# edouardoyallon/acco

Hardware: NVIDIA H100
Metric: tokens/sec (device-timed, max over ranks) Llama ACCO bf16 sharded-Adam, 8x1024 tokens per GPU per micro-batch (higher is better)
Workload: dtype bf16

## Files before the change

### acco_b200/csrc/bindings.cpp

```cpp
#include <torch/extension.h>
#include <ATen/cuda/CUDAContext.h>
#include <c10/cuda/CUDAGuard.h>
#include <cuda_runtime.h>

#include <cmath>
#include <cstdlib>
#include <vector>

extern "C" {
int acco_norm_grid(int T, int H, int sms, int backward);
int acco_rmsnorm_fwd(const void* a, const void* r, const void* w, void* y, void* h, float* rstd, int T, int H, float eps,
                     int grid, cudaStream_t st);
int acco_rmsnorm_bwd(const void* dy, const void* dh_extra, const void* h, const void* w, const float* rstd, void* dh,
                     float* dw_partial, float* dw_out, void* dw_accum_bf16, int T, int H, int grid, cudaStream_t st);
int acco_rope_pack_bwd(const void* dq, const void* dk, const void* dv, const long long* strides, void* dqkv, const float* cos_t,
                       const float* sin_t, int B, int S, int Hq, int Hk, int D, int sms, cudaStream_t st);
int acco_rope_qkv(void* qkv, const float* cos_t, const float* sin_t, int T, int S, int n_rot, int n_total, int D, int inverse,
                  int sms, cudaStream_t st);
int acco_swiglu_fwd(const void* gu, void* out, long long T, int I, int sms, cudaStream_t st);
int acco_swiglu_bwd(const void* dout, const void* gu, void* dgu, long long T, int I, int sms, cudaStream_t st);
int acco_ce_fwd(const void* logits, const long long* labels, float* lse, float* row_loss, float* loss, float* inv_n, long long T,
                int V, int Vp, long long ignore_index, cudaStream_t st);
int acco_ce_bwd(void* logits, const long long* labels, const float* lse, const float* scale, long long T, int V, int Vp,
                long long ignore_index, cudaStream_t st);
int acco_layernorm_grid(int T, int H, int sms, int backward);
int acco_layernorm_fwd(const void* a, const void* r, const void* w, const void* b, void* y, void* h, float* mean, float* rstd, int T, int H,
                       float eps, int grid, cudaStream_t st);
int acco_layernorm_bwd(const void* dy, const void* dh_extra, const void* h, const void* w, const float* mean, const float* rstd, void* dh,
                       float* partial, float* dwdb_out, void* dw_accum_bf16, void* db_accum_bf16, int T, int H, int grid, cudaStream_t st);
int acco_gelu_fwd(const void* x, void* y, long long n, int sms, cudaStream_t st);
int acco_gelu_bwd(const void* dy, const void* x, void* dx, long long n, int sms, cudaStream_t st);
int acco_debug_occupy(unsigned long long ns, int ctas, float* sink, cudaStream_t st);
int acco_round_params_size();
int acco_gemm_run(const void* a, long long lda, int a_mn, const void* b, long long ldb, int b_mn, void* d, long long ldd, const void* bias,
                  int M, int N, int K, int accumulate, int bn_req, int splits_req, int pm_req, int pn_req, int msub_req, int sms, cudaStream_t st);
int acco_gemm_tn_gather(const void* x, const void* w_local, void* y, int M, int N, int K, const void* const* peers, int n_peers,
                        const int* tile_owner, uint32_t* flags, uint32_t* epoch, uint32_t* done, int sms, cudaStream_t st);
long long acco_gemm_map_encodes();
int acco_gemm_max_clusters(int cl, int sms);
void acco_gemm_set_debug(unsigned long long* buf);
void acco_gemm_choose(int M, int N, int K, int a_mn, int b_mn, int accumulate, int sms, int* out5);
int acco_gemm_tile_n();
int acco_gemm_tile_k();
int acco_attn_supported(int B, int S, int Hq, int Hk, int D, float scale);
int acco_attn_fwd(const void* q, const void* k, const void* v, long long ld, void* o, long long ld_o, float* lse, int B, int S, int Hq, int Hk,
                  int D, float scale, int window, const int* seg, cudaStream_t st);
int acco_attn_bwd(const void* q, const void* k, const void* v, long long ld, const void* o, long long ld_o, const void* d_o, long long ld_do,
                  const float* lse, float* delta, float* dq_acc, void* dk, void* dv, int B, int S, int Hq, int Hk, int D, float scale, int window,
                  const int* seg, cudaStream_t st);
}

namespace {

constexpr int kMaxWorld = 16;
struct RoundParams {
    const void* acc_peer[kMaxWorld];
    void* theta_peer[kMaxWorld];
    uint32_t* pad_peer[kMaxWorld];
    const void* acc_mc;
    void* theta_mc;
    float* master;
    float* exp_avg;
    float* exp_avg_sq;
    float* stash;
    int* stash_count;
    int* total_out;
    uint32_t* epoch;
    uint32_t* done_ctas;
    const float* inv_count_in;
    const long long* skip;
    int n_skip;
    int watchdog_s;
    int gated;
    long long slice;
    int rank, world, local_count;
    float lr, beta1, beta2, eps, weight_decay, bc1, bc2_rsqrt;
    int commit, add_stash, write_stash;
};
extern "C" int acco_rs_adam_ag(const RoundParams* P, int grad_bf16, int out_bf16, int mode, int grid, cudaStream_t st);
extern "C" int acco_round_norm(const RoundParams* P, int grad_bf16, int mode, int grid, float max_norm, float* out, cudaStream_t st);

int sm_count() {
    static int n = 0;
    if (!n) n = at::cuda::getCurrentDeviceProperties()->multiProcessorCount;
    return n;
}
cudaStream_t stream() { return at::cuda::getCurrentCUDAStream().stream(); }

void check_bf16(const torch::Tensor& t, const char* name) {
    TORCH_CHECK(t.is_cuda() && t.scalar_type() == torch::kBFloat16 && t.is_contiguous(), name, " must be a contiguous CUDA bf16 tensor");
}
void check_f32(const torch::Tensor& t, const char* name) {
    TORCH_CHECK(t.is_cuda() && t.scalar_type() == torch::kFloat32 && t.is_contiguous(), name, " must be a contiguous CUDA fp32 tensor");
}

std::vector<torch::Tensor> rmsnorm_fwd(torch::Tensor x, torch::Tensor w, double eps) {
    check_bf16(x, "x"); check_bf16(w, "weight");
    const c10::cuda::CUDAGuard guard(x.device());
    const int T = x.size(0), H = x.size(1);
    auto y = torch::empty_like(x);
    auto rstd = torch::empty({T}, x.options().dtype(torch::kFloat32));
    const int grid = acco_norm_grid(T, H, sm_count(), 0);
    TORCH_CHECK(acco_rmsnorm_fwd(x.data_ptr(), nullptr, w.data_ptr(), y.data_ptr(), nullptr, rstd.data_ptr<float>(), T, H, (float)eps, grid, stream()) == 0,
                "rmsnorm_fwd: unsupported hidden size ", H);
    return {y, rstd};
}

std::vector<torch::Tensor> add_rmsnorm_fwd(torch::Tensor a, torch::Tensor r, torch::Tensor w, double eps) {
    check_bf16(a, "a"); check_bf16(r, "r"); check_bf16(w, "weight");
    const c10::cuda::CUDAGuard guard(a.device());
    const int T = a.size(0), H = a.size(1);
    auto y = torch::empty_like(a);
    auto h = torch::empty_like(a);
    auto rstd = torch::empty({T}, a.options().dtype(torch::kFloat32));
    const int grid = acco_norm_grid(T, H, sm_count(), 0);
    TORCH_CHECK(acco_rmsnorm_fwd(a.data_ptr(), r.data_ptr(), w.data_ptr(), y.data_ptr(), h.data_ptr(), rstd.data_ptr<float>(), T, H, (float)eps, grid, stream()) == 0,
                "add_rmsnorm_fwd: unsupported hidden size ", H);
    return {y, h, rstd};
}

std::vector<torch::Tensor> norm_bwd_impl(torch::Tensor dy, const torch::Tensor* de, torch::Tensor h, torch::Tensor w, torch::Tensor rstd,
                                         c10::optional<torch::Tensor> wgrad) {
    check_bf16(dy, "dy"); check_bf16(h, "h"); check_bf16(w, "weight"); check_f32(rstd, "rstd");
    const c10::cuda::CUDAGuard guard(dy.device());
    const int T = dy.size(0), H = dy.size(1);
    auto dh = torch::empty_like(dy);
    const int grid = acco_norm_grid(T, H, sm_count(), 1);
    auto partial = torch::empty({grid, H}, dy.options().dtype(torch::kFloat32));
    torch::Tensor dw;
    void* accum = nullptr;
    if (wgrad.has_value() && wgrad->defined()) {
        check_bf16(*wgrad, "weight.grad");
        TORCH_CHECK(wgrad->numel() == H, "weight.grad has the wrong size");
        accum = wgrad->data_ptr();
        dw = torch::empty({0}, dy.options().dtype(torch::kFloat32));
    } else {
        dw = torch::empty({H}, dy.options().dtype(torch::kFloat32));
    }
    TORCH_CHECK(acco_rmsnorm_bwd(dy.data_ptr(), de ? de->data_ptr() : nullptr, h.data_ptr(), w.data_ptr(), rstd.data_ptr<float>(), dh.data_ptr(),
                                 partial.data_ptr<float>(), accum ? nullptr : dw.data_ptr<float>(), accum, T, H, grid, stream()) == 0,
                "rmsnorm_bwd: unsupported hidden size ", H);
    return {dh, dw};
}
std::vector<torch::Tensor> rmsnorm_bwd(torch::Tensor dy, torch::Tensor x, torch::Tensor w, torch::Tensor rstd, c10::optional<torch::Tensor> wgrad) {
    return norm_bwd_impl(dy, nullptr, x, w, rstd, wgrad);
}
std::vector<torch::Tensor> add_rmsnorm_bwd(torch::Tensor dy, torch::Tensor dh_extra, torch::Tensor h, torch::Tensor w, torch::Tensor rstd,
                                           c10::optional<torch::Tensor> wgrad) {
    check_bf16(dh_extra, "dh_extra");
    return norm_bwd_impl(dy, &dh_extra, h, w, rstd, wgrad);
}

std::vector<torch::Tensor> layernorm_fwd(torch::Tensor a, c10::optional<torch::Tensor> r, torch::Tensor w, torch::Tensor b, double eps) {
    check_bf16(a, "a"); check_bf16(w, "weight"); check_bf16(b, "bias");
    const bool has_r = r.has_value() && r->defined();
    if (has_r) check_bf16(*r, "r");
    const c10::cuda::CUDAGuard guard(a.device());
    const int T = a.size(0), H = a.size(1);
    TORCH_CHECK(w.numel() == H && b.numel() == H, "layernorm: weight/bias size");
    auto y = torch::empty_like(a);
    auto f32 = a.options().dtype(torch::kFloat32);
    auto mean = torch::empty({T}, f32), rstd = torch::empty({T}, f32);
    torch::Tensor h = has_r ? torch::empty_like(a) : torch::Tensor();
    const int grid = acco_layernorm_grid(T, H, sm_count(), 0);
    TORCH_CHECK(acco_layernorm_fwd(a.data_ptr(), has_r ? r->data_ptr() : nullptr, w.data_ptr(), b.data_ptr(), y.data_ptr(), has_r ? h.data_ptr() : nullptr,
                                   mean.data_ptr<float>(), rstd.data_ptr<float>(), T, H, (float)eps, grid, stream()) == 0,
                "layernorm_fwd: unsupported hidden size ", H);
    if (has_r) return {y, h, mean, rstd};
    return {y, mean, rstd};
}

std::vector<torch::Tensor> layernorm_bwd(torch::Tensor dy, c10::optional<torch::Tensor> dh_extra, torch::Tensor h, torch::Tensor w, torch::Tensor mean,
                                         torch::Tensor rstd, c10::optional<torch::Tensor> wgrad, c10::optional<torch::Tensor> bgrad) {
    check_bf16(dy, "dy"); check_bf16(h, "h"); check_bf16(w, "weight"); check_f32(mean, "mean"); check_f32(rstd, "rstd");
    const bool has_e = dh_extra.has_value() && dh_extra->defined();
    if (has_e) check_bf16(*dh_extra, "dh_extra");
    const c10::cuda::CUDAGuard guard(dy.device());
    const int T = dy.size(0), H = dy.size(1);
    auto dh = torch::empty_like(dy);
    const int grid = acco_layernorm_grid(T, H, sm_count(), 1);
    auto f32 = dy.options().dtype(torch::kFloat32);
    auto partial = torch::empty({grid, 2 * H}, f32);
    const bool accum = wgrad.has_value() && wgrad->defined() && bgrad.has_value() && bgrad->defined();
    torch::Tensor dwdb;
    if (accum) {
        check_bf16(*wgrad, "weight.grad"); check_bf16(*bgrad, "bias.grad");
        TORCH_CHECK(wgrad->numel() == H && bgrad->numel() == H, "grad sizes");
        dwdb = torch::empty({0}, f32);
    } else {
        dwdb = torch::empty({2 * H}, f32);
    }
    TORCH_CHECK(acco_layernorm_bwd(dy.data_ptr(), has_e ? dh_extra->data_ptr() : nullptr, h.data_ptr(), w.data_ptr(), mean.data_ptr<float>(),
                                   rstd.data_ptr<float>(), dh.data_ptr(), partial.data_ptr<float>(), accum ? nullptr : dwdb.data_ptr<float>(),
                                   accum ? wgrad->data_ptr() : nullptr, accum ? bgrad->data_ptr() : nullptr, T, H, grid, stream()) == 0,
                "layernorm_bwd: unsupported hidden size ", H);
    return {dh, dwdb};
}

torch::Tensor gelu_fwd(torch::Tensor x) {
    check_bf16(x, "x");
    const c10::cuda::CUDAGuard guard(x.device());
    auto y = torch::empty_like(x);
    TORCH_CHECK(acco_gelu_fwd(x.data_ptr(), y.data_ptr(), x.numel(), sm_count(), stream()) == 0, "gelu: numel must be a multiple of 8");
    return y;
}
torch::Tensor gelu_bwd(torch::Tensor dy, torch::Tensor x) {
    check_bf16(x, "x"); check_bf16(dy, "dy");
    const c10::cuda::CUDAGuard guard(x.device());
    auto dx = torch::empty_like(x);
    TORCH_CHECK(acco_gelu_bwd(dy.data_ptr(), x.data_ptr(), dx.data_ptr(), x.numel(), sm_count(), stream()) == 0, "gelu: numel must be a multiple of 8");
    return dx;
}

void rope_qkv_inplace(torch::Tensor qkv, torch::Tensor cos_t, torch::Tensor sin_t, int64_t B, int64_t S, int64_t n_rot,
                      int64_t n_total, int64_t D, bool inverse) {
    check_bf16(qkv, "qkv"); check_f32(cos_t, "cos"); check_f32(sin_t, "sin");
    const c10::cuda::CUDAGuard guard(qkv.device());
    TORCH_CHECK(qkv.numel() == B * S * n_total * D, "qkv has the wrong number of elements");
    TORCH_CHECK(cos_t.size(0) >= S && cos_t.size(1) == D / 2, "cos/sin tables must be [>=S, D/2]");
    TORCH_CHECK(acco_rope_qkv(qkv.data_ptr(), cos_t.data_ptr<float>(), sin_t.data_ptr<float>(), (int)(B * S), (int)S, (int)n_rot,
                              (int)n_total, (int)D, inverse ? 1 : 0, sm_count(), stream()) == 0,
                "rope: head_dim must be a multiple of 16");
}

torch::Tensor rope_pack_bwd(torch::Tensor dq, torch::Tensor dk, torch::Tensor dv, torch::Tensor cos_t, torch::Tensor sin_t) {
    TORCH_CHECK(dq.is_cuda() && dq.scalar_type() == torch::kBFloat16 && dk.scalar_type() == torch::kBFloat16 && dv.scalar_type() == torch::kBFloat16, "bf16 CUDA grads expected");
    TORCH_CHECK(dq.stride(3) == 1 && dk.stride(3) == 1 && dv.stride(3) == 1, "head dim must be contiguous");
    check_f32(cos_t, "cos"); check_f32(sin_t, "sin");
    const c10::cuda::CUDAGuard guard(dq.device());
    const int64_t B = dq.size(0), S = dq.size(1), Hq = dq.size(2), D = dq.size(3), Hk = dk.size(2);
    for (auto* t : {&dq, &dk, &dv}) TORCH_CHECK((t->stride(0) % 8 == 0) && (t->stride(1) % 8 == 0) && (t->stride(2) % 8 == 0) && ((uintptr_t)t->data_ptr() % 16 == 0), "16-byte aligned strides required");
    auto out = torch::empty({B * S, (Hq + 2 * Hk) * D}, dq.options());
    long long st[9] = {dq.stride(0), dq.stride(1), dq.stride(2), dk.stride(0), dk.stride(1), dk.stride(2), dv.stride(0), dv.stride(1), dv.stride(2)};
    TORCH_CHECK(acco_rope_pack_bwd(dq.data_ptr(), dk.data_ptr(), dv.data_ptr(), st, out.data_ptr(), cos_t.data_ptr<float>(), sin_t.data_ptr<float>(),
                                   (int)B, (int)S, (int)Hq, (int)Hk, (int)D, sm_count(), stream()) == 0, "rope_pack_bwd: head_dim must be a multiple of 16");
    return out;
}

torch::Tensor swiglu_fwd(torch::Tensor gu) {
    check_bf16(gu, "gate_up");
    const c10::cuda::CUDAGuard guard(gu.device());
    const int64_t T = gu.size(0), I = gu.size(1) / 2;
    auto out = torch::empty({T, I}, gu.options());
    TORCH_CHECK(acco_swiglu_fwd(gu.data_ptr(), out.data_ptr(), T, (int)I, sm_count(), stream()) == 0, "swiglu: I must be a multiple of 8");
    return out;
}

torch::Tensor swiglu_bwd(torch::Tensor dout, torch::Tensor gu) {
    check_bf16(dout, "dout"); check_bf16(gu, "gate_up");
    const c10::cuda::CUDAGuard guard(gu.device());
    const int64_t T = gu.size(0), I = gu.size(1) / 2;
    auto dgu = torch::empty_like(gu);
    TORCH_CHECK(acco_swiglu_bwd(dout.data_ptr(), gu.data_ptr(), dgu.data_ptr(), T, (int)I, sm_count(), stream()) == 0, "swiglu: I must be a multiple of 8");
    return dgu;
}

std::vector<torch::Tensor> ce_fwd(torch::Tensor logits, torch::Tensor labels, int64_t V, int64_t ignore_index) {
    check_bf16(logits, "logits");
    TORCH_CHECK(labels.is_cuda() && labels.scalar_type() == torch::kInt64 && labels.is_contiguous(), "labels must be contiguous CUDA int64");
    const c10::cuda::CUDAGuard guard(logits.device());
    const int64_t T = logits.size(0), Vp = logits.size(1);
    TORCH_CHECK(labels.numel() == T, "labels/logits row mismatch");
    auto f32 = logits.options().dtype(torch::kFloat32);
    auto lse = torch::empty({T}, f32);
    auto row_loss = torch::empty({T}, f32);
    auto loss = torch::empty({}, f32);
    auto inv_n = torch::empty({1}, f32);
    TORCH_CHECK(acco_ce_fwd(logits.data_ptr(), (const long long*)labels.data_ptr<int64_t>(), lse.data_ptr<float>(), row_loss.data_ptr<float>(),
                            loss.data_ptr<float>(), inv_n.data_ptr<float>(), T, (int)V, (int)Vp, ignore_index, stream()) == 0,
                "ce_fwd: padded vocab must be a multiple of 8 and >= V");
    return {loss, inv_n, lse};
}

void ce_bwd_inplace(torch::Tensor logits, torch::Tensor labels, torch::Tensor lse, torch::Tensor scale, int64_t V, int64_t ignore_index) {
    check_bf16(logits, "logits"); check_f32(lse, "lse"); check_f32(scale, "scale");
    const c10::cuda::CUDAGuard guard(logits.device());
    const int64_t T = logits.size(0), Vp = logits.size(1);
    TORCH_CHECK(acco_ce_bwd(logits.data_ptr(), (const long long*)labels.data_ptr<int64_t>(), lse.data_ptr<float>(), scale.data_ptr<float>(), T,
                            (int)V, (int)Vp, ignore_index, stream()) == 0, "ce_bwd: bad shapes");
}

int default_grid(int mode, long long slice) {
    const long long vec = slice / 8;
    long long want = (vec + 255) / 256;
    long long cap = mode == 0 ? (long long)sm_count() * 4 : (long long)sm_count();
    if (want < 1) want = 1;
    return (int)std::min(want, cap);
}

void fill_hyper(RoundParams& P, double lr, double b1, double b2, double eps, double wd, int64_t step, int64_t commit, bool add_stash, bool write_stash) {
    P.lr = (float)lr; P.beta1 = (float)b1; P.beta2 = (float)b2; P.eps = (float)eps; P.weight_decay = (float)wd;
    P.bc1 = (float)(1.0 - std::pow(b1, (double)step));
    P.bc2_rsqrt = (float)(1.0 / std::sqrt(1.0 - std::pow(b2, (double)step)));
    P.commit = (int)commit; P.add_stash = add_stash ? 1 : 0; P.write_stash = write_stash ? 1 : 0;
}

void adamw_shard(torch::Tensor grad_sum, torch::Tensor master, torch::Tensor exp_avg, torch::Tensor exp_avg_sq, torch::Tensor stash,
                 torch::Tensor out, torch::Tensor inv_count, torch::Tensor scratch ,
                 double lr, double b1, double b2, double eps, double wd, int64_t step, int64_t commit, bool add_stash, bool write_stash) {
    check_f32(master, "master"); check_f32(exp_avg, "exp_avg"); check_f32(exp_avg_sq, "exp_avg_sq"); check_f32(stash, "stash"); check_f32(inv_count, "inv_count");
    const c10::cuda::CUDAGuard guard(master.device());
    const int64_t S = master.numel();
    TORCH_CHECK(S % 8 == 0, "shard size must be a multiple of 8 (use slice alignment >= 8)");
    TORCH_CHECK(grad_sum.numel() >= S && out.numel() >= S && grad_sum.is_contiguous() && out.is_contiguous(), "bad grad/out");
    TORCH_CHECK(scratch.scalar_type() == torch::kInt32 && scratch.numel() >= 4, "scratch must be int32[4]");
    const bool gb = grad_sum.scalar_type() == torch::kBFloat16, ob = out.scalar_type() == torch::kBFloat16;
    TORCH_CHECK(gb || grad_sum.scalar_type() == torch::kFloat32, "grad dtype");
    TORCH_CHECK(ob || out.scalar_type() == torch::kFloat32, "out dtype");
    RoundParams P{};
    P.acc_peer[0] = grad_sum.data_ptr();
    P.theta_peer[0] = out.data_ptr();
    P.master = master.data_ptr<float>(); P.exp_avg = exp_avg.data_ptr<float>(); P.exp_avg_sq = exp_avg_sq.data_ptr<float>(); P.stash = stash.data_ptr<float>();
    int* sc = scratch.data_ptr<int>();
    P.stash_count = sc; P.total_out = sc + 1; P.epoch = (uint32_t*)(sc + 2); P.done_ctas = (uint32_t*)(sc + 3);
    P.inv_count_in = inv_count.data_ptr<float>();
    P.slice = S; P.rank = 0; P.world = 1; P.local_count = 0;
    fill_hyper(P, lr, b1, b2, eps, wd, step, commit, add_stash, write_stash);
    TORCH_CHECK(acco_rs_adam_ag(&P, gb, ob, 0, default_grid(0, S), stream()) == 0, "adamw_shard launch failed");
}

RoundParams round_params(const std::vector<int64_t>& acc_ptrs, const std::vector<int64_t>& theta_ptrs, const std::vector<int64_t>& pad_ptrs,
                         int64_t acc_mc, int64_t theta_mc, const torch::Tensor& stash, const torch::Tensor& scratch, int64_t slice, int64_t rank,
                         int64_t world, int64_t local_count, int64_t mode) {
    check_f32(stash, "stash");
    TORCH_CHECK(world >= 1 && world <= kMaxWorld, "world size out of range");
    TORCH_CHECK(mode >= 0 && mode <= 2, "mode must be 0 (local), 1 (p2p) or 2 (multimem)");
    TORCH_CHECK((int64_t)acc_ptrs.size() >= (mode == 0 ? 1 : world), "peer pointer table too short");
    TORCH_CHECK(mode == 0 || (int64_t)pad_ptrs.size() >= world, "signal pad table too short");
    TORCH_CHECK(slice % 8 == 0 && stash.numel() == slice, "slice must be a multiple of 8 and match the shard state");
    TORCH_CHECK(mode != 2 || acc_mc != 0, "multicast mode needs multicast pointers");
    TORCH_CHECK(scratch.scalar_type() == torch::kInt32 && scratch.numel() >= 4, "scratch must be int32[4]");
    RoundParams P{};
    for (size_t i = 0; i < acc_ptrs.size() && i < (size_t)kMaxWorld; ++i) P.acc_peer[i] = (const void*)acc_ptrs[i];
    for (size_t i = 0; i < theta_ptrs.size() && i < (size_t)kMaxWorld; ++i) P.theta_peer[i] = (void*)theta_ptrs[i];
    for (size_t i = 0; i < pad_ptrs.size() && i < (size_t)kMaxWorld; ++i) P.pad_peer[i] = (uint32_t*)pad_ptrs[i];
    P.acc_mc = (const void*)acc_mc; P.theta_mc = (void*)theta_mc;
    P.stash = stash.data_ptr<float>();
    int* sc = scratch.data_ptr<int>();
    P.stash_count = sc; P.total_out = sc + 1; P.epoch = (uint32_t*)(sc + 2); P.done_ctas = (uint32_t*)(sc + 3);
    P.inv_count_in = nullptr;
    P.slice = slice; P.rank = (int)rank; P.world = (int)world; P.local_count = (int)local_count;
    static int watchdog = -1;
    if (watchdog < 0) { const char* e = std::getenv("ACCO_ROUND_WATCHDOG_S"); watchdog = e ? std::atoi(e) : 1800; }
    P.watchdog_s = watchdog;
    static int gated = -1;
    if (gated < 0) { const char* e = std::getenv("ACCO_ROUND_GATE"); gated = (e && e[0] == '0') ? 0 : 1; }
    P.gated = mode != 0 ? gated : 0;
    return P;
}

void rs_adam_ag(std::vector<int64_t> acc_ptrs, std::vector<int64_t> theta_ptrs, std::vector<int64_t> pad_ptrs, int64_t acc_mc, int64_t theta_mc,
                torch::Tensor master, torch::Tensor exp_avg, torch::Tensor exp_avg_sq, torch::Tensor stash,
                torch::Tensor scratch , int64_t slice, int64_t rank, int64_t world, int64_t local_count,
                double lr, double b1, double b2, double eps, double wd, int64_t step, int64_t commit, bool add_stash, bool write_stash,
                bool grad_bf16, bool out_bf16, int64_t mode, int64_t grid, c10::optional<torch::Tensor> skip_ranges,
                c10::optional<torch::Tensor> inv_count) {
    check_f32(master, "master"); check_f32(exp_avg, "exp_avg"); check_f32(exp_avg_sq, "exp_avg_sq");
    const c10::cuda::CUDAGuard guard(master.device());
    TORCH_CHECK(master.numel() == slice, "slice must match the shard state");
    TORCH_CHECK((int64_t)theta_ptrs.size() >= (mode == 0 ? 1 : world), "peer pointer tables too short");
    TORCH_CHECK(mode != 2 || theta_mc != 0, "multicast mode needs multicast pointers");
    RoundParams P = round_params(acc_ptrs, theta_ptrs, pad_ptrs, acc_mc, theta_mc, stash, scratch, slice, rank, world, local_count, mode);
    P.master = master.data_ptr<float>(); P.exp_avg = exp_avg.data_ptr<float>(); P.exp_avg_sq = exp_avg_sq.data_ptr<float>();
    if (skip_ranges.has_value() && skip_ranges->defined() && skip_ranges->numel() > 0) {
        TORCH_CHECK(skip_ranges->is_cuda() && skip_ranges->scalar_type() == torch::kInt64 && skip_ranges->is_contiguous() && skip_ranges->numel() % 2 == 0,
                    "skip_ranges must be a contiguous CUDA int64 [n, 2] tensor");
        P.skip = (const long long*)skip_ranges->data_ptr<int64_t>();
        P.n_skip = (int)(skip_ranges->numel() / 2);
    }
    if (inv_count.has_value() && inv_count->defined()) {
        check_f32(*inv_count, "inv_count");
        TORCH_CHECK(inv_count->numel() >= 2, "inv_count must be the scratch of round_norm (inv_eff at index 1)");
        P.inv_count_in = inv_count->data_ptr<float>() + 1;
        if (mode != 0) P.gated = 2;
    }
    fill_hyper(P, lr, b1, b2, eps, wd, step, commit, add_stash, write_stash);
    const int g = grid > 0 ? (int)grid : default_grid((int)mode, slice);
    TORCH_CHECK(acco_rs_adam_ag(&P, grad_bf16, out_bf16, (int)mode, g, stream()) == 0, "rs_adam_ag launch failed");
}

void round_norm(std::vector<int64_t> acc_ptrs, std::vector<int64_t> pad_ptrs, int64_t acc_mc, torch::Tensor stash, torch::Tensor scratch,
                torch::Tensor out, int64_t slice, int64_t rank, int64_t world, int64_t local_count, bool add_stash, bool grad_bf16, int64_t mode,
                int64_t grid, double max_norm) {
    check_f32(out, "out");
    const c10::cuda::CUDAGuard guard(stash.device());
    TORCH_CHECK(max_norm > 0, "max_norm must be positive");
    RoundParams P = round_params(acc_ptrs, std::vector<int64_t>(), pad_ptrs, acc_mc, 0, stash, scratch, slice, rank, world, local_count, mode);
    P.add_stash = add_stash ? 1 : 0;
    const int g = grid > 0 ? (int)grid : default_grid((int)mode, slice);
    TORCH_CHECK(out.numel() >= 3 + g, "out must hold 3 + grid floats (", 3 + g, ")");
    TORCH_CHECK(acco_round_norm(&P, grad_bf16, (int)mode, g, (float)max_norm, out.data_ptr<float>(), stream()) == 0, "round_norm launch failed");
}

torch::Tensor gemm_tn(torch::Tensor x, torch::Tensor w, std::vector<int64_t> peer_ptrs, c10::optional<torch::Tensor> tile_owner,
                      c10::optional<torch::Tensor> flags, c10::optional<torch::Tensor> state, int64_t max_ctas) {
    check_bf16(x, "x"); check_bf16(w, "w");
    TORCH_CHECK(x.dim() == 2 && w.dim() == 2 && x.size(1) == w.size(1), "gemm_tn: x [M,K], w [N,K]");
    const c10::cuda::CUDAGuard guard(x.device());
    const int64_t M = x.size(0), K = x.size(1), N = w.size(0);
    TORCH_CHECK(K % 8 == 0 && N % 8 == 0, "gemm_tn: K and N must be multiples of 8");
    TORCH_CHECK((uintptr_t)x.data_ptr() % 16 == 0 && (uintptr_t)w.data_ptr() % 16 == 0, "gemm_tn: 16-byte aligned operands required");
    auto y = torch::empty({M, N}, x.options());
    const void* peers[8] = {nullptr};
    const int n_peers = (int)peer_ptrs.size();
    TORCH_CHECK(n_peers <= 8, "gemm_tn: at most 8 peers");
    const int* owner = nullptr; uint32_t* fl = nullptr; uint32_t* ep = nullptr; uint32_t* dn = nullptr;
    if (n_peers > 0) {
        TORCH_CHECK(tile_owner.has_value() && flags.has_value() && state.has_value(), "gather mode needs tile_owner, flags and state");
        const int64_t num_n = (N + acco_gemm_tile_n() - 1) / acco_gemm_tile_n(), num_k = (K + acco_gemm_tile_k() - 1) / acco_gemm_tile_k();
        TORCH_CHECK(tile_owner->scalar_type() == torch::kInt32 && tile_owner->numel() >= num_n && tile_owner->is_cuda(), "tile_owner: int32 CUDA [num_n]");
        TORCH_CHECK(flags->scalar_type() == torch::kInt32 && flags->numel() >= num_n * num_k * 2 && flags->is_cuda(), "flags: int32 CUDA [num_n*num_k*2]");
        TORCH_CHECK(state->scalar_type() == torch::kInt32 && state->numel() >= 2 && state->is_cuda(), "state: int32 CUDA [2]");
        for (int i = 0; i < n_peers; ++i) peers[i] = (const void*)peer_ptrs[i];
        owner = tile_owner->data_ptr<int>();
        fl = (uint32_t*)flags->data_ptr<int>();
        ep = (uint32_t*)state->data_ptr<int>();
        dn = ep + 1;
    }
    int sms = sm_count();
    if (max_ctas > 0 && max_ctas < sms) sms = (int)max_ctas;
    int rc;
    if (n_peers > 0)
        rc = acco_gemm_tn_gather(x.data_ptr(), w.data_ptr(), y.data_ptr(), (int)M, (int)N, (int)K, peers, n_peers, owner, fl, ep, dn, sms, stream());
    else
        rc = acco_gemm_run(x.data_ptr(), K, 0, w.data_ptr(), K, 0, y.data_ptr(), N, nullptr, (int)M, (int)N, (int)K, 0, 0, 0, 0, 0, 0, sms, stream());
    TORCH_CHECK(rc == 0, "gemm_tn launch failed, code ", rc);
    return y;
}

torch::Tensor gemm(torch::Tensor a, torch::Tensor b, c10::optional<torch::Tensor> out, c10::optional<torch::Tensor> bias, bool a_mn, bool b_mn,
                   bool accumulate, int64_t bn, int64_t splits, int64_t pm, int64_t pn, int64_t msub, int64_t max_ctas) {
    auto ok2d = [](const torch::Tensor& t) {
        return t.is_cuda() && t.scalar_type() == torch::kBFloat16 && t.dim() == 2 && t.stride(1) == 1 && t.stride(0) % 8 == 0 && t.stride(0) >= t.size(1) &&
               (uintptr_t)t.data_ptr() % 16 == 0;
    };
    TORCH_CHECK(ok2d(a) && ok2d(b), "gemm: operands must be 2-D CUDA bf16, unit inner stride, 16-byte aligned rows");
    const c10::cuda::CUDAGuard guard(a.device());
    const int64_t M = a_mn ? a.size(1) : a.size(0), K = a_mn ? a.size(0) : a.size(1);
    const int64_t N = b_mn ? b.size(1) : b.size(0), Kb = b_mn ? b.size(0) : b.size(1);
    TORCH_CHECK(K == Kb, "gemm: contraction sizes differ (", K, " vs ", Kb, ")");
    TORCH_CHECK(N % 8 == 0, "gemm: N must be a multiple of 8");
    torch::Tensor y;
    if (out.has_value() && out->defined()) {
        y = *out;
        TORCH_CHECK(ok2d(y) && y.size(0) == M && y.size(1) == N, "gemm: out must be a [M,N] CUDA bf16 matrix");
    } else {
        TORCH_CHECK(!accumulate, "gemm: accumulate needs `out`");
        y = torch::empty({M, N}, a.options());
    }
    const void* bias_p = nullptr;
    if (bias.has_value() && bias->defined()) {
        TORCH_CHECK(bias->is_cuda() && bias->scalar_type() == torch::kBFloat16 && bias->is_contiguous() && bias->numel() == N &&
                    (uintptr_t)bias->data_ptr() % 16 == 0, "gemm: bias must be a contiguous, 16-byte aligned CUDA bf16 [N] vector");
        bias_p = bias->data_ptr();
    }
    int sms = sm_count();
    if (max_ctas > 0 && max_ctas < sms) sms = (int)max_ctas;
    const int rc = acco_gemm_run(a.data_ptr(), a.stride(0), a_mn ? 1 : 0, b.data_ptr(), b.stride(0), b_mn ? 1 : 0, y.data_ptr(), y.stride(0), bias_p,
                             (int)M, (int)N, (int)K, accumulate ? 1 : 0, (int)bn, (int)splits, (int)pm, (int)pn, (int)msub, sms, stream());
    TORCH_CHECK(rc == 0, "gemm launch failed, code ", rc, " (M=", M, " N=", N, " K=", K, ")");
    return y;
}

std::vector<int64_t> gemm_choose(int64_t M, int64_t N, int64_t K, bool a_mn, bool b_mn, bool accumulate) {
    int o[5] = {0, 0, 0, 0, 0};
    acco_gemm_choose((int)M, (int)N, (int)K, a_mn ? 1 : 0, b_mn ? 1 : 0, accumulate ? 1 : 0, sm_count(), o);
    return {o[0], o[1], o[2], o[3], o[4]};
}
int64_t gemm_map_encodes() { return acco_gemm_map_encodes(); }
void gemm_set_debug(c10::optional<torch::Tensor> buf) {
    if (buf.has_value() && buf->defined()) {
        TORCH_CHECK(buf->is_cuda() && buf->scalar_type() == torch::kInt64 && buf->numel() >= 16 && buf->is_contiguous(), "int64 CUDA [16] expected");
        acco_gemm_set_debug((unsigned long long*)buf->data_ptr<int64_t>());
    } else {
        acco_gemm_set_debug(nullptr);
    }
}
int64_t gemm_max_clusters(int64_t cl) { return acco_gemm_max_clusters((int)cl, sm_count()); }

int64_t num_sms() { return sm_count(); }

int64_t prefer_shared_carveout() { return (int64_t)cudaDeviceSetCacheConfig(cudaFuncCachePreferShared); }

bool attn_supported(int64_t B, int64_t S, int64_t Hq, int64_t Hk, int64_t D, double scale) {
    return acco_attn_supported((int)B, (int)S, (int)Hq, (int)Hk, (int)D, (float)scale) != 0;
}
static void check_rows(const torch::Tensor& t, int64_t rows, int64_t cols, const char* name) {
    TORCH_CHECK(t.is_cuda() && t.scalar_type() == torch::kBFloat16 && t.dim() == 2 && t.size(0) == rows && t.size(1) == cols && t.stride(1) == 1 &&
                t.stride(0) % 8 == 0 && (uintptr_t)t.data_ptr() % 16 == 0, name, " must be a [", rows, ", ", cols, "] CUDA bf16 matrix with 16-byte aligned rows");
}
static const int* seg_ptr(const c10::optional<torch::Tensor>& seg, int64_t B, int64_t S) {
    if (!seg.has_value() || !seg->defined()) return nullptr;
    TORCH_CHECK(seg->is_cuda() && seg->scalar_type() == torch::kInt32 && seg->is_contiguous() && seg->numel() == B * S,
                "seg must be a contiguous CUDA int32 tensor of B*S segment starts");
    return seg->data_ptr<int>();
}
std::vector<torch::Tensor> attn_fwd(torch::Tensor qkv, int64_t B, int64_t S, int64_t Hq, int64_t Hk, int64_t D, double scale, int64_t window,
                                    c10::optional<torch::Tensor> seg) {
    check_rows(qkv, B * S, (Hq + 2 * Hk) * D, "qkv");
    const c10::cuda::CUDAGuard guard(qkv.device());
    auto o = torch::empty({B * S, Hq * D}, qkv.options());
    auto lse = torch::empty({B, Hq, S}, qkv.options().dtype(torch::kFloat32));
    const auto* base = (const char*)qkv.data_ptr();
    const int rc = acco_attn_fwd(base, base + 2 * Hq * D, base + 2 * (Hq + Hk) * D, qkv.stride(0), o.data_ptr(), o.stride(0), lse.data_ptr<float>(), (int)B, (int)S,
                                 (int)Hq, (int)Hk, (int)D, (float)scale, (int)window, seg_ptr(seg, B, S), stream());
    TORCH_CHECK(rc == 0, "attn_fwd launch failed, code ", rc, " (B=", B, " S=", S, " Hq=", Hq, " Hk=", Hk, " D=", D, ")");
    return {o, lse};
}
std::vector<torch::Tensor> attn_bwd(torch::Tensor qkv, torch::Tensor o, torch::Tensor d_o, torch::Tensor lse, int64_t B, int64_t S, int64_t Hq, int64_t Hk,
                                    int64_t D, double scale, int64_t window, c10::optional<torch::Tensor> seg) {
    check_rows(qkv, B * S, (Hq + 2 * Hk) * D, "qkv");
    check_rows(o, B * S, Hq * D, "o");
    check_rows(d_o, B * S, Hq * D, "d_o");
    check_f32(lse, "lse");
    TORCH_CHECK(lse.numel() == B * Hq * S, "lse must be [B, Hq, S]");
    const c10::cuda::CUDAGuard guard(qkv.device());
    auto f32 = qkv.options().dtype(torch::kFloat32);
    auto delta = torch::empty({B, Hq, S}, f32);
    auto dq = torch::empty({B * S, Hq * D}, f32);
    auto dk = torch::empty({B * S, Hk * D}, qkv.options());
    auto dv = torch::empty({B * S, Hk * D}, qkv.options());
    const auto* base = (const char*)qkv.data_ptr();
    const int rc = acco_attn_bwd(base, base + 2 * Hq * D, base + 2 * (Hq + Hk) * D, qkv.stride(0), o.data_ptr(), o.stride(0), d_o.data_ptr(), d_o.stride(0),
                                 lse.data_ptr<float>(), delta.data_ptr<float>(), dq.data_ptr<float>(), dk.data_ptr(), dv.data_ptr(), (int)B, (int)S, (int)Hq,
                                 (int)Hk, (int)D, (float)scale, (int)window, seg_ptr(seg, B, S), stream());
    TORCH_CHECK(rc == 0, "attn_bwd launch failed, code ", rc);
    return {dq, dk, dv};
}

void debug_occupy(double us, int64_t ctas, torch::Tensor sink) {
    check_f32(sink, "sink");
    const c10::cuda::CUDAGuard guard(sink.device());
    TORCH_CHECK(acco_debug_occupy((unsigned long long)(us * 1e3), (int)ctas, sink.data_ptr<float>(), stream()) == 0, "occupy launch failed");
}

}

torch::Tensor pack_const_len_native(torch::Tensor flat_tokens, torch::Tensor doc_lens, int64_t max_length, int64_t eos);

PYBIND11_MODULE(TORCH_EXTENSION_NAME, m) {
    TORCH_CHECK(acco_round_params_size() == (int)sizeof(RoundParams), "RoundParams layout mismatch between bindings.cpp and rs_adam_ag.cu");
    m.def("rmsnorm_fwd", &rmsnorm_fwd);
    m.def("rmsnorm_bwd", &rmsnorm_bwd);
    m.def("add_rmsnorm_fwd", &add_rmsnorm_fwd);
    m.def("add_rmsnorm_bwd", &add_rmsnorm_bwd);
    m.def("layernorm_fwd", &layernorm_fwd);
    m.def("layernorm_bwd", &layernorm_bwd);
    m.def("gelu_fwd", &gelu_fwd);
    m.def("gelu_bwd", &gelu_bwd);
    m.def("rope_qkv_inplace", &rope_qkv_inplace);
    m.def("rope_pack_bwd", &rope_pack_bwd);
    m.def("swiglu_fwd", &swiglu_fwd);
    m.def("swiglu_bwd", &swiglu_bwd);
    m.def("ce_fwd", &ce_fwd);
    m.def("ce_bwd_inplace", &ce_bwd_inplace);
    m.def("adamw_shard", &adamw_shard);
    m.def("rs_adam_ag", &rs_adam_ag, py::arg("acc_ptrs"), py::arg("theta_ptrs"), py::arg("pad_ptrs"), py::arg("acc_mc"), py::arg("theta_mc"),
          py::arg("master"), py::arg("exp_avg"), py::arg("exp_avg_sq"), py::arg("stash"), py::arg("scratch"), py::arg("slice"), py::arg("rank"),
          py::arg("world"), py::arg("local_count"), py::arg("lr"), py::arg("b1"), py::arg("b2"), py::arg("eps"), py::arg("wd"), py::arg("step"),
          py::arg("commit"), py::arg("add_stash"), py::arg("write_stash"), py::arg("grad_bf16"), py::arg("out_bf16"), py::arg("mode"),
          py::arg("grid"), py::arg("skip_ranges"), py::arg("inv_count") = py::none());
    m.def("round_norm", &round_norm, py::arg("acc_ptrs"), py::arg("pad_ptrs"), py::arg("acc_mc"), py::arg("stash"), py::arg("scratch"),
          py::arg("out"), py::arg("slice"), py::arg("rank"), py::arg("world"), py::arg("local_count"), py::arg("add_stash"), py::arg("grad_bf16"),
          py::arg("mode"), py::arg("grid"), py::arg("max_norm"));
    m.def("gemm_tn", &gemm_tn);
    m.def("gemm", &gemm);
    m.def("gemm_choose", &gemm_choose);
    m.def("gemm_map_encodes", &gemm_map_encodes);
    m.def("gemm_max_clusters", &gemm_max_clusters);
    m.def("gemm_set_debug", &gemm_set_debug);
    m.def("num_sms", &num_sms);
    m.def("prefer_shared_carveout", &prefer_shared_carveout);
    m.def("attn_supported", &attn_supported);
    m.def("attn_fwd", &attn_fwd, py::arg("qkv"), py::arg("B"), py::arg("S"), py::arg("Hq"), py::arg("Hk"), py::arg("D"), py::arg("scale"),
          py::arg("window"), py::arg("seg") = py::none());
    m.def("attn_bwd", &attn_bwd, py::arg("qkv"), py::arg("o"), py::arg("d_o"), py::arg("lse"), py::arg("B"), py::arg("S"), py::arg("Hq"),
          py::arg("Hk"), py::arg("D"), py::arg("scale"), py::arg("window"), py::arg("seg") = py::none());
    m.def("debug_occupy", &debug_occupy);
    m.def("pack_const_len", &pack_const_len_native);
}
```

### acco_b200/csrc/elementwise.cu

```cuda
#include <stdlib.h>

#include "common.cuh"

namespace acco {

ACCO_DEVINL void load_cs(const float* __restrict__ cos_t, const float* __restrict__ sin_t, int pos, int half, int v, float (&c)[8],
                         float (&s)[8]) {
    const float4* cp = reinterpret_cast<const float4*>(cos_t + (size_t)pos * half + 8 * v);
    const float4* sp = reinterpret_cast<const float4*>(sin_t + (size_t)pos * half + 8 * v);
    const float4 c0 = __ldg(cp), c1 = __ldg(cp + 1), s0 = __ldg(sp), s1 = __ldg(sp + 1);
    c[0] = c0.x; c[1] = c0.y; c[2] = c0.z; c[3] = c0.w; c[4] = c1.x; c[5] = c1.y; c[6] = c1.z; c[7] = c1.w;
    s[0] = s0.x; s[1] = s0.y; s[2] = s0.z; s[3] = s0.w; s[4] = s1.x; s[5] = s1.y; s[6] = s1.z; s[7] = s1.w;
}

__global__ void __launch_bounds__(256) rope_qkv_kernel(__nv_bfloat16* __restrict__ qkv, const float* __restrict__ cos_t,
                                                       const float* __restrict__ sin_t, int T, int S, int n_rot,
                                                       int n_total, int D, float sign) {
    const int half = D >> 1;
    const int vph = half >> 3;
    const int lane = threadIdx.x & 31;
    const int v = lane % vph, hg = lane / vph, hstep = 32 / vph;
    const int warps = (gridDim.x * blockDim.x) >> 5;
    for (int t = (blockIdx.x * blockDim.x + threadIdx.x) >> 5; t < T; t += warps) {
        float c[8], s[8];
        load_cs(cos_t, sin_t, t % S, half, v, c, s);
        __nv_bfloat16* row = qkv + (size_t)t * n_total * D + 8 * v;
        for (int h = hg; h < n_rot; h += hstep) {
            __nv_bfloat16* p1 = row + (size_t)h * D;
            float x1[8], x2[8], o1[8], o2[8];
            unpack8(ld_vec(p1), x1);
            unpack8(ld_vec(p1 + half), x2);
#pragma unroll
            for (int j = 0; j < 8; ++j) {
                const float sj = sign * s[j];
                o1[j] = x1[j] * c[j] - x2[j] * sj;
                o2[j] = x2[j] * c[j] + x1[j] * sj;
            }
            st_vec(p1, pack8(o1));
            st_vec(p1 + half, pack8(o2));
        }
    }
}

struct PackSrc {
    const __nv_bfloat16* ptr[3];
    long long sb[3], ss[3], sh[3];
};
__global__ void __launch_bounds__(256) rope_pack_bwd_kernel(PackSrc src, __nv_bfloat16* __restrict__ dqkv,
                                                            const float* __restrict__ cos_t, const float* __restrict__ sin_t,
                                                            int B, int S, int Hq, int Hk, int D) {
    const int half = D >> 1;
    const int vph = half >> 3;
    const int n_total = Hq + 2 * Hk;
    const int lane = threadIdx.x & 31;
    const int v = lane % vph, hg = lane / vph, hstep = 32 / vph;
    const int warps = (gridDim.x * blockDim.x) >> 5;
    const int T = B * S;
    for (int t = (blockIdx.x * blockDim.x + threadIdx.x) >> 5; t < T; t += warps) {
        const int s = t % S, b = t / S;
        float c[8], sn[8];
        load_cs(cos_t, sin_t, s, half, v, c, sn);
        __nv_bfloat16* orow = dqkv + (size_t)t * n_total * D + 8 * v;
        for (int head = hg; head < n_total; head += hstep) {
            int which, h;
            if (head < Hq) { which = 0; h = head; }
            else if (head < Hq + Hk) { which = 1; h = head - Hq; }
            else { which = 2; h = head - Hq - Hk; }
            const __nv_bfloat16* p1 = src.ptr[which] + b * src.sb[which] + s * src.ss[which] + h * src.sh[which] + 8 * v;
            float x1[8], x2[8];
            unpack8(ld_stream(p1), x1);
            unpack8(ld_stream(p1 + half), x2);
            __nv_bfloat16* o1 = orow + (size_t)head * D;
            if (which == 2) {
                st_vec(o1, pack8(x1));
                st_vec(o1 + half, pack8(x2));
            } else {
                float r1[8], r2[8];
#pragma unroll
                for (int j = 0; j < 8; ++j) {
                    r1[j] = x1[j] * c[j] + x2[j] * sn[j];
                    r2[j] = x2[j] * c[j] - x1[j] * sn[j];
                }
                st_vec(o1, pack8(r1));
                st_vec(o1 + half, pack8(r2));
            }
        }
    }
}

__global__ void __launch_bounds__(256) swiglu_fwd_kernel(const __nv_bfloat16* __restrict__ gu, __nv_bfloat16* __restrict__ out,
                                                         long long T, int I) {
    const int vpr = I >> 3;
    const long long total = T * vpr;
    for (long long idx = (long long)blockIdx.x * blockDim.x + threadIdx.x; idx < total;
         idx += (long long)gridDim.x * blockDim.x) {
        const long long t = idx / vpr;
        const int v = (int)(idx % vpr);
        const __nv_bfloat16* g = gu + t * 2 * I + 8 * v;
        float fg[8], fu[8], o[8];
        unpack8(ld_stream(g), fg);
        unpack8(ld_stream(g + I), fu);
#pragma unroll
        for (int j = 0; j < 8; ++j) {
            const float sg = 1.f / (1.f + __expf(-fg[j]));
            o[j] = fg[j] * sg * fu[j];
        }
        st_stream(out + t * I + 8 * v, pack8(o));
    }
}

__global__ void __launch_bounds__(256) swiglu_bwd_kernel(const __nv_bfloat16* __restrict__ dout,
                                                         const __nv_bfloat16* __restrict__ gu, __nv_bfloat16* __restrict__ dgu,
                                                         long long T, int I) {
    const int vpr = I >> 3;
    const long long total = T * vpr;
    for (long long idx = (long long)blockIdx.x * blockDim.x + threadIdx.x; idx < total;
         idx += (long long)gridDim.x * blockDim.x) {
        const long long t = idx / vpr;
        const int v = (int)(idx % vpr);
        const __nv_bfloat16* g = gu + t * 2 * I + 8 * v;
        float fg[8], fu[8], fd[8], dg[8], du[8];
        unpack8(ld_stream(g), fg);
        unpack8(ld_stream(g + I), fu);
        unpack8(ld_stream(dout + t * I + 8 * v), fd);
#pragma unroll
        for (int j = 0; j < 8; ++j) {
            const float sg = 1.f / (1.f + __expf(-fg[j]));
            const float silu = fg[j] * sg;
            dg[j] = fd[j] * fu[j] * sg * (1.f + fg[j] * (1.f - sg));
            du[j] = fd[j] * silu;
        }
        __nv_bfloat16* o = dgu + t * 2 * I + 8 * v;
        st_stream(o, pack8(dg));
        st_stream(o + I, pack8(du));
    }
}

static int grid_for(long long work_items, int threads, int sms) {
    long long want = (work_items + threads - 1) / threads;
    long long cap = (long long)sms * (2048 / threads) * 4;
    if (want < 1) want = 1;
    return (int)(want < cap ? want : cap);
}

}

extern "C" int acco_rope_qkv(void* qkv, const float* cos_t, const float* sin_t, int T, int S, int n_rot, int n_total, int D,
                             int inverse, int sms, cudaStream_t st) {
    if (D % 16 != 0 || (32 % (D / 16)) != 0) return -1;
    const long long work = (long long)T * 32;
    acco::rope_qkv_kernel<<<acco::grid_for(work, 256, sms), 256, 0, st>>>((__nv_bfloat16*)qkv, cos_t, sin_t, T, S, n_rot,
                                                                          n_total, D, inverse ? -1.f : 1.f);
    return 0;
}

extern "C" int acco_rope_pack_bwd(const void* dq, const void* dk, const void* dv, const long long* strides ,
                                  void* dqkv, const float* cos_t, const float* sin_t, int B, int S, int Hq, int Hk, int D, int sms,
                                  cudaStream_t st) {
    if (D % 16 != 0 || (32 % (D / 16)) != 0) return -1;
    acco::PackSrc src;
    src.ptr[0] = (const __nv_bfloat16*)dq; src.ptr[1] = (const __nv_bfloat16*)dk; src.ptr[2] = (const __nv_bfloat16*)dv;
    for (int i = 0; i < 3; ++i) { src.sb[i] = strides[3 * i]; src.ss[i] = strides[3 * i + 1]; src.sh[i] = strides[3 * i + 2]; }
    const long long work = (long long)B * S * 32;
    acco::rope_pack_bwd_kernel<<<acco::grid_for(work, 256, sms), 256, 0, st>>>(src, (__nv_bfloat16*)dqkv, cos_t, sin_t, B, S, Hq, Hk, D);
    return 0;
}

extern "C" int acco_swiglu_fwd(const void* gu, void* out, long long T, int I, int sms, cudaStream_t st) {
    if (I % 8 != 0) return -1;
    acco::swiglu_fwd_kernel<<<acco::grid_for(T * (I / 8), 256, sms), 256, 0, st>>>((const __nv_bfloat16*)gu,
                                                                                    (__nv_bfloat16*)out, T, I);
    return 0;
}

extern "C" int acco_swiglu_bwd(const void* dout, const void* gu, void* dgu, long long T, int I, int sms, cudaStream_t st) {
    if (I % 8 != 0) return -1;
    acco::swiglu_bwd_kernel<<<acco::grid_for(T * (I / 8), 256, sms), 256, 0, st>>>(
        (const __nv_bfloat16*)dout, (const __nv_bfloat16*)gu, (__nv_bfloat16*)dgu, T, I);
    return 0;
}

namespace acco {
__global__ void __launch_bounds__(256, 4) occupy_kernel(unsigned long long ns, float* sink) {
    float v[56];
#pragma unroll
    for (int i = 0; i < 56; ++i) v[i] = (float)(threadIdx.x + i);
    unsigned long long t0, t;
    asm volatile("mov.u64 %0, %%globaltimer;" : "=l"(t0));
    do {
#pragma unroll
        for (int i = 0; i < 56; ++i) v[i] = v[i] * 1.0001f + v[(i + 7) % 56];
        __nanosleep(200);
        asm volatile("mov.u64 %0, %%globaltimer;" : "=l"(t));
    } while (t - t0 < ns);
    float s = 0.f;
#pragma unroll
    for (int i = 0; i < 56; ++i) s += v[i];
    if (s == 123.456f) sink[0] = s;
}
}

extern "C" int acco_debug_occupy(unsigned long long ns, int ctas, float* sink, cudaStream_t st) {
    static bool once = false;
    if (!once) {
        const char* e = getenv("ACCO_OCCUPY_DEFAULT_CARVEOUT");
        if (!(e && e[0] == '1')) cudaFuncSetAttribute(acco::occupy_kernel, cudaFuncAttributePreferredSharedMemoryCarveout, cudaSharedmemCarveoutMaxShared);
        once = true;
    }
    acco::occupy_kernel<<<ctas, 256, 0, st>>>(ns, sink);
    return (int)cudaGetLastError();
}
```

### acco_b200/csrc/gemm_wgmma.cu

```cuda
#include <cuda.h>
#include <cuda_bf16.h>
#include <cuda_runtime.h>
#include <stdint.h>
#include <stdlib.h>

#include <mutex>
#include <unordered_map>

#include "wgmma.cuh"

namespace acco_gemm {

using namespace acco_tc;

constexpr int BM = 128, BN_MAX = 256, BK = 64;
constexpr int A_BYTES = BM * BK * 2;
constexpr int RING_BYTES = 192 * 1024;
constexpr int MAX_STAGES = 8;
constexpr int EPI_BUF_BYTES = 64 * 64 * 2;
constexpr int EPI_BYTES = 2 * 2 * EPI_BUF_BYTES;
constexpr int SMEM_BYTES = RING_BYTES + EPI_BYTES + 1024  + 256 ;
constexpr int THREADS = 384;
constexpr int MAX_PEERS = 8;
constexpr int MN_CHUNK_BYTES = 64 * BK * 2;

struct Params {
    CUtensorMap map_a;
    CUtensorMap map_b;
    CUtensorMap map_b_peer[MAX_PEERS];
    CUtensorMap map_d;
    const __nv_bfloat16* bias;
    const int* tile_owner;
    uint32_t* flags;
    uint32_t* epoch;
    uint32_t* done_ctas;
    __nv_bfloat16* out;
    long long ldd;
    int M, N, K;
    int splits, kb_per_split;
    int reduce;
    int atomic;
    int gather;
    int stages, stage_bytes;
    int pm, pn;
    int band;
    unsigned long long* dbg;
};

__device__ __forceinline__ void wait_flag_gpu(const uint32_t* f, uint32_t epoch) {
    uint32_t v;
    unsigned spins = 0;
    unsigned long long t0 = 0;
    do {
        asm volatile("ld.acquire.gpu.global.u32 %0, [%1];" : "=r"(v) : "l"(f) : "memory");
        if ((++spins & 0xFFFFF) == 0) {
            unsigned long long now;
            asm volatile("mov.u64 %0, %%globaltimer;" : "=l"(now));
            if (t0 == 0) t0 = now;
            else if (now - t0 > 60ull * 1000000000ull) __trap();
        }
    } while ((int32_t)(v - epoch) < 0);
}

__device__ __forceinline__ void stamp(const Params& P, int slot) {
    if (P.dbg != nullptr && blockIdx.x == 0) {
        unsigned long long t;
        asm volatile("mov.u64 %0, %%globaltimer;" : "=l"(t));
        P.dbg[slot] = t;
    }
}

struct Unit {
    int mb, n_blk, kb0, kb1;
};
__device__ __forceinline__ Unit decode_unit(int t, int tiles, int num_smb, int num_sn, int band, int num_k, int kb_per_split, int pm, int pn,
                                            int pi, int pj) {
    Unit u;
    const int s = t / tiles, tile = t - s * tiles;
    const int bi = tile / (band * num_smb), sn0 = bi * band;
    const int width = min(band, num_sn - sn0);
    const int r = tile - sn0 * num_smb;
    const int smb = r / width;
    u.mb = smb * pm + pi;
    u.n_blk = (sn0 + r - smb * width) * pn + pj;
    u.kb0 = s * kb_per_split;
    u.kb1 = min(num_k, u.kb0 + kb_per_split);
    return u;
}

template <int BN, int TA, int TB>
__device__ __forceinline__ void mma_k16(float (&acc)[BN / 2], uint64_t da, uint64_t db, uint32_t scale_d) {
    if constexpr (BN == 256) wgmma_m64n256k16<TA, TB>(acc, da, db, scale_d);
    else if constexpr (BN == 128) wgmma_m64n128k16<TA, TB>(acc, da, db, scale_d);
    else wgmma_m64n64k16<TA, TB>(acc, da, db, scale_d);
}

template <int BN, int A_MN, int B_MN>
__global__ void __launch_bounds__(THREADS, 1) gemm_kernel(const __grid_constant__ Params P) {
    extern __shared__ uint8_t smem_raw[];
    if (threadIdx.x == 0) stamp(P, 0);
    uint8_t* smem = (uint8_t*)(((uintptr_t)smem_raw + 1023) & ~(uintptr_t)1023);
    uint8_t* epi_smem = smem + RING_BYTES;
    uint64_t* full_bar = (uint64_t*)(epi_smem + EPI_BYTES);
    uint64_t* empty_bar = full_bar + MAX_STAGES;
    uint64_t* c_bar = empty_bar + MAX_STAGES;

    constexpr int B_BYTES = BN * BK * 2;
    const int wg = threadIdx.x >> 7, tid = threadIdx.x & 127;
    const int n_stages = P.stages, stage_bytes = P.stage_bytes;
    const int pm = P.pm, pn = P.pn, cl_size = pm * pn;
    const uint32_t cl_rank = cl_size > 1 ? cluster_ctarank() : 0u;
    const int pi = (int)cl_rank / pn, pj = (int)cl_rank - pi * pn;
    const int unit0 = blockIdx.x / cl_size, unit_stride = gridDim.x / cl_size;
    const int num_n = (P.N + BN - 1) / BN, num_k = (P.K + BK - 1) / BK, num_mb = (P.M + BM - 1) / BM;
    const int num_sn = (num_n + pn - 1) / pn, num_smb = (num_mb + pm - 1) / pm;
    const int band = P.band;
    const int tiles = num_smb * num_sn;
    const int num_units = tiles * P.splits;
    const int kbs = P.kb_per_split;
    uint16_t mask_a = 0, mask_b = 0;
    for (int j = 0; j < pn; ++j) mask_a |= (uint16_t)(1u << (pi * pn + j));
    for (int i = 0; i < pm; ++i) mask_b |= (uint16_t)(1u << (i * pn + pj));
    const uint16_t mask_rel = mask_a | mask_b;

    if (threadIdx.x == 0) {
        asm volatile("prefetch.tensormap [%0];" ::"l"(&P.map_a) : "memory");
        asm volatile("prefetch.tensormap [%0];" ::"l"(&P.map_b) : "memory");
        asm volatile("prefetch.tensormap [%0];" ::"l"(&P.map_d) : "memory");
        for (int s = 0; s < n_stages; ++s) {
            mbar_init(&full_bar[s], 1);
            mbar_init(&empty_bar[s], 2u * (uint32_t)(pm + pn - 1));
        }
        for (int b = 0; b < 4; ++b) mbar_init(&c_bar[b], 1);
        asm volatile("fence.mbarrier_init.release.cluster;" ::: "memory");
    }
    __syncthreads();
    if (cl_size > 1) cluster_sync_all();
    if (threadIdx.x == 0) stamp(P, 1);
    asm volatile("griddepcontrol.wait;" ::: "memory");
    asm volatile("griddepcontrol.launch_dependents;" ::: "memory");
    if (threadIdx.x == 0) stamp(P, 2);
    const uint32_t epoch = P.gather ? (*(volatile uint32_t*)P.epoch + 1u) : 0u;
    auto flag_ptr = [&](int n_blk, int kb, int half) { return P.flags + ((size_t)n_blk * num_k + kb) * 2 + half; };

    if (wg == 0) {
        asm volatile("setmaxnreg.dec.sync.aligned.u32 40;");
        if (tid == 0) {
            int stage = 0;
            uint32_t phase = 0;
            const int a_rows = BM / pn, a_off = pj * a_rows;
            const int nach = (BM / 64) / pn, a_ch0 = pj * nach;
            const int b_rows = BN / pm, b_off = pi * b_rows;
            const int nbch = (BN / 64) / pm, b_ch0 = pi * nbch;
            const bool mc_a = pn > 1, mc_b = pm > 1;
            for (int t = unit0; t < num_units; t += unit_stride) {
                const Unit u = decode_unit(t, tiles, num_smb, num_sn, band, num_k, kbs, pm, pn, pi, pj);
                const int n_blk = u.n_blk;
                const int m0 = u.mb * BM, n0 = n_blk * BN;
                const int owner = P.gather ? P.tile_owner[n_blk] : -1;
                const bool gatherer = owner >= 0 && u.mb == 0;
                const bool waiter = owner >= 0 && u.mb != 0;
                const CUtensorMap* bmap = gatherer ? &P.map_b_peer[owner] : &P.map_b;
                bool all_ready = !waiter;
                if (waiter) {
                    uint32_t v0, v1;
                    asm volatile("ld.acquire.gpu.global.u32 %0, [%1];" : "=r"(v0) : "l"(flag_ptr(n_blk, num_k - 1, 0)) : "memory");
                    asm volatile("ld.acquire.gpu.global.u32 %0, [%1];" : "=r"(v1) : "l"(flag_ptr(n_blk, num_k - 1, 1)) : "memory");
                    all_ready = (int32_t)(v0 - epoch) >= 0 && (int32_t)(v1 - epoch) >= 0;
                    if (all_ready) asm volatile("fence.proxy.async;" ::: "memory");
                }
                for (int kb = u.kb0; kb < u.kb1; ++kb) {
                    if (!all_ready) {
                        wait_flag_gpu(flag_ptr(n_blk, kb, 0), epoch);
                        wait_flag_gpu(flag_ptr(n_blk, kb, 1), epoch);
                        asm volatile("fence.proxy.async;" ::: "memory");
                    }
                    mbar_wait(&empty_bar[stage], phase ^ 1);
                    uint8_t* sa = smem + stage * stage_bytes;
                    uint8_t* sb = sa + A_BYTES;
                    mbar_expect_tx(&full_bar[stage], (uint32_t)(A_BYTES + B_BYTES));
                    if (A_MN) {
                        for (int c = a_ch0; c < a_ch0 + nach; ++c) {
                            if (mc_a) tma_load_2d_mc(&P.map_a, &full_bar[stage], sa + c * MN_CHUNK_BYTES, m0 + c * 64, kb * BK, mask_a);
                            else tma_load_2d(&P.map_a, &full_bar[stage], sa + c * MN_CHUNK_BYTES, m0 + c * 64, kb * BK);
                        }
                    } else {
                        if (mc_a) tma_load_2d_mc(&P.map_a, &full_bar[stage], sa + a_off * 128, kb * BK, m0 + a_off, mask_a);
                        else tma_load_2d(&P.map_a, &full_bar[stage], sa, kb * BK, m0);
                    }
                    if (B_MN) {
                        for (int c = b_ch0; c < b_ch0 + nbch; ++c) {
                            if (mc_b) tma_load_2d_mc(bmap, &full_bar[stage], sb + c * MN_CHUNK_BYTES, n0 + c * 64, kb * BK, mask_b);
                            else tma_load_2d(bmap, &full_bar[stage], sb + c * MN_CHUNK_BYTES, n0 + c * 64, kb * BK);
                        }
                    } else {
                        if (mc_b) tma_load_2d_mc(bmap, &full_bar[stage], sb + b_off * 128, kb * BK, n0 + b_off, mask_b);
                        else tma_load_2d(bmap, &full_bar[stage], sb, kb * BK, n0);
                    }
                    if (gatherer) {
                        mbar_wait(&full_bar[stage], phase);
                        fence_async_smem();
                        tma_store_2d(&P.map_b, sb, kb * BK, n0);
                        asm volatile("cp.async.bulk.commit_group;" ::: "memory");
                        asm volatile("cp.async.bulk.wait_group 0;" ::: "memory");
                        asm volatile("fence.proxy.async;" ::: "memory");
                        asm volatile("st.release.gpu.global.u32 [%0], %1;" ::"l"(flag_ptr(n_blk, kb, 0)), "r"(epoch) : "memory");
                        asm volatile("st.release.gpu.global.u32 [%0], %1;" ::"l"(flag_ptr(n_blk, kb, 1)), "r"(epoch) : "memory");
                    }
                    if (t == unit0 && kb == u.kb0) stamp(P, 3);
                    if (++stage == n_stages) { stage = 0; phase ^= 1; }
                }
            }
            stamp(P, 9);
        }
    } else {
        asm volatile("setmaxnreg.inc.sync.aligned.u32 232;");
        const int cw = wg - 1;
        const int warp = tid >> 5, lane = tid & 31;
        const bool releaser = cl_size > 1 ? (tid < 16 && ((mask_rel >> tid) & 1)) : tid == 0;
        constexpr uint32_t a_lbo = A_MN ? (MN_CHUNK_BYTES >> 4) : 1, a_sbo = 1024 >> 4, a_kstep = A_MN ? 2048 : 32;
        constexpr uint32_t b_lbo = B_MN ? (MN_CHUNK_BYTES >> 4) : 1, b_sbo = 1024 >> 4, b_kstep = B_MN ? 2048 : 32;
        auto release = [&](int s) {
            if (!releaser) return;
            if (cl_size > 1) mbar_arrive_cluster_addr(map_to_cta(&empty_bar[s], (uint32_t)tid));
            else mbar_arrive(&empty_bar[s]);
        };
        constexpr int NSUB = BN / 64;
        constexpr int NPRE = NSUB < 2 ? NSUB : 2;
        uint8_t* epi = epi_smem + cw * 2 * EPI_BUF_BYTES;
        uint64_t* cbar = c_bar + cw * 2;
        const bool load_c = P.reduce && !P.atomic;
        const int bar_id = 1 + cw;
        uint32_t c_phase = 0;
        auto wait_buffer_free = [&]() {
            if (NSUB == 1) bulk_wait_read<0>();
            else bulk_wait_read<1>();
        };
        auto load_c_sub = [&](const Unit& u, int s) {
            mbar_expect_tx(&cbar[s & 1], (uint32_t)EPI_BUF_BYTES);
            tma_load_2d(&P.map_d, &cbar[s & 1], epi + (s & 1) * EPI_BUF_BYTES, u.n_blk * BN + s * 64, u.mb * BM + cw * 64);
        };
        float acc[BN / 2];
#pragma unroll
        for (int i = 0; i < BN / 2; ++i) acc[i] = 0.f;
        int stage = 0;
        uint32_t phase = 0;
        for (int t = unit0; t < num_units; t += unit_stride) {
            const Unit u = decode_unit(t, tiles, num_smb, num_sn, band, num_k, kbs, pm, pn, pi, pj);
            int prev = -1;
            for (int kb = u.kb0; kb < u.kb1; ++kb) {
                mbar_wait(&full_bar[stage], phase);
                if (cw == 0 && tid == 0 && t == unit0 && kb == u.kb0) stamp(P, 4);
                const uint32_t a_addr = smem_u32(smem + stage * stage_bytes) + (uint32_t)(cw * 8192);
                const uint32_t b_addr = smem_u32(smem + stage * stage_bytes + A_BYTES);
                wgmma_fence();
#pragma unroll
                for (int k = 0; k < BK / 16; ++k) {
                    const uint64_t da = make_smem_desc(a_addr + k * a_kstep, a_lbo, a_sbo);
                    const uint64_t db = make_smem_desc(b_addr + k * b_kstep, b_lbo, b_sbo);
                    mma_k16<BN, A_MN, B_MN>(acc, da, db, (uint32_t)((kb > u.kb0) | (k != 0)));
                }
                wgmma_commit();
                if (load_c && kb == u.kb0 && tid == 0) {
                    bulk_wait_read<0>();
                    for (int s = 0; s < NPRE; ++s) load_c_sub(u, s);
                }
                if (prev >= 0) {
                    wgmma_wait<1>();
                    release(prev);
                }
                prev = stage;
                if (++stage == n_stages) { stage = 0; phase ^= 1; }
            }
            wgmma_wait<0>();
            reg_fence(acc);
            release(prev);
            const int m0 = u.mb * BM + cw * 64;
            const uint32_t row_addr = smem_u32(epi) + (uint32_t)((warp * 16 + (lane >> 2)) * 128 + 4 * (lane & 3));
            const int colb = u.n_blk * BN + 2 * (lane & 3);
            const bool bias_on = P.bias != nullptr && u.kb0 == 0;
#pragma unroll
            for (int s = 0; s < NSUB; ++s) {
                uint8_t* buf = epi + (s & 1) * EPI_BUF_BYTES;
                const uint32_t buf_addr = row_addr + (uint32_t)((s & 1) * EPI_BUF_BYTES);
                if (load_c) {
                    if (s >= NPRE && tid == 0) {
                        wait_buffer_free();
                        load_c_sub(u, s);
                    }
                    mbar_wait(&cbar[s & 1], (c_phase >> (s & 1)) & 1u);
                    c_phase ^= 1u << (s & 1);
                } else {
                    if (tid == 0) wait_buffer_free();
                    named_barrier(bar_id, 128);
                }
#pragma unroll
                for (int jj = 0; jj < 8; ++jj) {
                    const int j = s * 8 + jj;
                    const int col = colb + 8 * j;
                    float b0 = 0.f, b1 = 0.f;
                    if (bias_on && col < P.N) {
                        const float2 f = __bfloat1622float2(*reinterpret_cast<const __nv_bfloat162*>(P.bias + col));
                        b0 = f.x; b1 = f.y;
                    }
                    const uint32_t chunk_addr = buf_addr + (uint32_t)((jj ^ (lane >> 2)) << 4);
#pragma unroll
                    for (int h = 0; h < 2; ++h) {
                        const uint32_t dst = chunk_addr + h * 8 * 128;
                        float v0 = acc[4 * j + 2 * h] + b0, v1 = acc[4 * j + 2 * h + 1] + b1;
                        if (load_c) {
                            const uint32_t cv = ld_shared_u32(dst);
                            const float2 c = __bfloat1622float2(*reinterpret_cast<const __nv_bfloat162*>(&cv));
                            v0 += c.x; v1 += c.y;
                        }
                        st_shared_u32(dst, pack_bf16x2(v0, v1));
                    }
                }
                fence_async_smem();
                named_barrier(bar_id, 128);
                if (tid == 0) {
                    if (P.atomic) tma_reduce_add_2d(&P.map_d, buf, u.n_blk * BN + s * 64, m0);
                    else tma_store_2d(&P.map_d, buf, u.n_blk * BN + s * 64, m0);
                    bulk_commit();
                }
            }
        }
        if (tid == 0) bulk_wait<0>();
        if (cw == 0 && tid == 0) stamp(P, 7);
    }

    __syncthreads();
    if (threadIdx.x == 0) stamp(P, 10);
    if (cl_size > 1) cluster_sync_all();
    if (P.gather && threadIdx.x == 0) {
        __threadfence();
        const uint32_t prev = atomicAdd(P.done_ctas, 1u);
        if (prev == gridDim.x - 1) {
            *P.done_ctas = 0;
            __threadfence();
            *P.epoch = epoch;
        }
    }
}

typedef CUresult (*EncodeFn)(CUtensorMap*, CUtensorMapDataType, cuuint32_t, void*, const cuuint64_t*, const cuuint64_t*, const cuuint32_t*,
                             const cuuint32_t*, CUtensorMapInterleave, CUtensorMapSwizzle, CUtensorMapL2promotion, CUtensorMapFloatOOBfill);

static EncodeFn get_encode() {
    static EncodeFn fn = nullptr;
    static std::once_flag once;
    std::call_once(once, [] {
        void* p = nullptr;
        cudaDriverEntryPointQueryResult q;
        if (cudaGetDriverEntryPoint("cuTensorMapEncodeTiled", &p, cudaEnableDefault, &q) == cudaSuccess) fn = (EncodeFn)p;
    });
    return fn;
}

static bool bind_primary_context() {
    typedef CUresult (*DeviceGetFn)(CUdevice*, int);
    typedef CUresult (*RetainFn)(CUcontext*, CUdevice);
    typedef CUresult (*SetCurrentFn)(CUcontext);
    void *p_get = nullptr, *p_retain = nullptr, *p_set = nullptr;
    cudaDriverEntryPointQueryResult q;
    if (cudaGetDriverEntryPoint("cuDeviceGet", &p_get, cudaEnableDefault, &q) != cudaSuccess ||
        cudaGetDriverEntryPoint("cuDevicePrimaryCtxRetain", &p_retain, cudaEnableDefault, &q) != cudaSuccess ||
        cudaGetDriverEntryPoint("cuCtxSetCurrent", &p_set, cudaEnableDefault, &q) != cudaSuccess)
        return false;
    int dev = 0;
    CUdevice d;
    CUcontext c = nullptr;
    if (cudaGetDevice(&dev) != cudaSuccess || ((DeviceGetFn)p_get)(&d, dev) != CUDA_SUCCESS) return false;
    return ((RetainFn)p_retain)(&c, d) == CUDA_SUCCESS && ((SetCurrentFn)p_set)(c) == CUDA_SUCCESS;
}

struct MapKey {
    const void* base;
    uint64_t inner, outer, ld;
    uint32_t box_inner, box_outer;
    int elem_bytes;
    bool operator==(const MapKey& o) const {
        return base == o.base && inner == o.inner && outer == o.outer && ld == o.ld && box_inner == o.box_inner && box_outer == o.box_outer &&
               elem_bytes == o.elem_bytes;
    }
};
struct MapKeyHash {
    size_t operator()(const MapKey& k) const {
        size_t h = (size_t)k.base;
        auto mix = [&h](uint64_t v) { h ^= v + 0x9e3779b97f4a7c15ull + (h << 6) + (h >> 2); };
        mix(k.inner); mix(k.outer); mix(k.ld); mix(((uint64_t)k.box_inner << 32) | k.box_outer); mix((uint64_t)k.elem_bytes);
        return h;
    }
};
static std::mutex g_map_mu;
static std::unordered_map<MapKey, CUtensorMap, MapKeyHash> g_maps;
static long long g_map_encodes = 0;

int make_map_typed(CUtensorMap* m, const void* base, uint64_t inner, uint64_t outer, uint64_t ld, uint32_t box_inner, uint32_t box_outer,
                   int elem_bytes) {
    const MapKey key{base, inner, outer, ld, box_inner, box_outer, elem_bytes};
    {
        std::lock_guard<std::mutex> g(g_map_mu);
        auto it = g_maps.find(key);
        if (it != g_maps.end()) { *m = it->second; return 0; }
    }
    EncodeFn enc = get_encode();
    if (!enc) return -2;
    cuuint64_t dims[2] = {inner, outer};
    cuuint64_t strides[1] = {ld * (uint64_t)elem_bytes};
    cuuint32_t box[2] = {box_inner, box_outer};
    cuuint32_t estr[2] = {1, 1};
    CUresult r = enc(m, elem_bytes == 4 ? CU_TENSOR_MAP_DATA_TYPE_FLOAT32 : CU_TENSOR_MAP_DATA_TYPE_BFLOAT16, 2, const_cast<void*>(base), dims, strides, box, estr, CU_TENSOR_MAP_INTERLEAVE_NONE,
                     CU_TENSOR_MAP_SWIZZLE_128B, CU_TENSOR_MAP_L2_PROMOTION_L2_256B, CU_TENSOR_MAP_FLOAT_OOB_FILL_NONE);
    if (r == CUDA_ERROR_INVALID_CONTEXT && bind_primary_context()) {
        r = enc(m, elem_bytes == 4 ? CU_TENSOR_MAP_DATA_TYPE_FLOAT32 : CU_TENSOR_MAP_DATA_TYPE_BFLOAT16, 2, const_cast<void*>(base), dims, strides, box, estr,
                CU_TENSOR_MAP_INTERLEAVE_NONE, CU_TENSOR_MAP_SWIZZLE_128B, CU_TENSOR_MAP_L2_PROMOTION_L2_256B, CU_TENSOR_MAP_FLOAT_OOB_FILL_NONE);
    }
    if (r != CUDA_SUCCESS) return -3;
    std::lock_guard<std::mutex> g(g_map_mu);
    if (g_maps.size() > 8192) g_maps.clear();
    g_maps.emplace(key, *m);
    ++g_map_encodes;
    return 0;
}
static int make_map(CUtensorMap* m, const void* base, uint64_t inner, uint64_t outer, uint64_t ld, uint32_t box_inner, uint32_t box_outer) {
    return make_map_typed(m, base, inner, outer, ld, box_inner, box_outer, 2);
}

typedef void (*KernelFn)(const Params);
template <int BN>
static KernelFn kernel_for(int a_mn, int b_mn) {
    if (a_mn) return b_mn ? gemm_kernel<BN, 1, 1> : gemm_kernel<BN, 1, 0>;
    return b_mn ? gemm_kernel<BN, 0, 1> : gemm_kernel<BN, 0, 0>;
}
static KernelFn kernel_for(int bn, int a_mn, int b_mn) {
    if (bn == 256) return kernel_for<256>(a_mn, b_mn);
    if (bn == 128) return kernel_for<128>(a_mn, b_mn);
    return kernel_for<64>(a_mn, b_mn);
}

static int g_pm = 0, g_pn = 0;
static unsigned long long* g_dbg = nullptr;
static int g_pdl = 1;
static int init_once() {
    static int rc = 0;
    static std::once_flag once;
    std::call_once(once, [] {
        for (int bn : {64, 128, 256})
            for (int a = 0; a < 2; ++a)
                for (int b = 0; b < 2; ++b)
                    if (cudaFuncSetAttribute(kernel_for(bn, a, b), cudaFuncAttributeMaxDynamicSharedMemorySize, SMEM_BYTES) != cudaSuccess) rc = -4;
        const char* e;
        if ((e = getenv("ACCO_GEMM_CLUSTER")) && e[0] && e[1] == ',') { g_pm = e[0] - '0'; g_pn = e[2] - '0'; }
        if ((e = getenv("ACCO_GEMM_PDL")) && e[0] == '0') g_pdl = 0;
    });
    return rc;
}

static int max_clusters(int cl, int sms) {
    static int cache[17] = {0};
    static std::mutex mu;
    std::lock_guard<std::mutex> g(mu);
    if (cl < 2 || cl > 16) return sms;
    if (!cache[cl]) {
        cudaLaunchConfig_t cfg = {};
        cfg.gridDim = dim3(cl * 64);
        cfg.blockDim = dim3(THREADS);
        cfg.dynamicSmemBytes = SMEM_BYTES;
        cudaLaunchAttribute attr[1];
        attr[0].id = cudaLaunchAttributeClusterDimension;
        attr[0].val.clusterDim.x = cl;
        attr[0].val.clusterDim.y = 1;
        attr[0].val.clusterDim.z = 1;
        cfg.attrs = attr;
        cfg.numAttrs = 1;
        int n = 0;
        if (cudaOccupancyMaxActiveClusters(&n, gemm_kernel<256, 0, 0>, &cfg) != cudaSuccess || n <= 0) { cudaGetLastError(); n = -1; }
        cache[cl] = n;
    }
    const int n = cache[cl];
    if (n <= 0) return 0;
    return n < sms / cl ? n : sms / cl;
}

struct Config {
    int bn, splits, pm, pn;
};

static Config choose_config(int M, int N, int K, int a_mn, int b_mn, int reduce, int sms, int bn_req, int splits_req, int pm_req, int pn_req) {
    (void)a_mn; (void)b_mn;
    const int num_k = (K + BK - 1) / BK;
    double best = 1e30;
    Config bc{256, 1, 1, 1};
    const int cands[3] = {256, 128, 64};
    const int num_mb = (M + BM - 1) / BM;
    for (int ci = 0; ci < 3; ++ci) {
        const int bn = cands[ci];
        if (bn_req > 0 && bn != bn_req) continue;
        if (bn_req <= 0 && bn > 64 && bn / 2 >= N) continue;
        const int num_n = (N + bn - 1) / bn;
        for (int pm = 1; pm <= 2; ++pm) {
            for (int pn = 1; pn <= 2; ++pn) {
                if ((pm_req > 0 && pm != pm_req) || (pm_req <= 0 && pm != 1)) continue;
                if ((pn_req > 0 && pn != pn_req) || (pn_req <= 0 && pn != 1)) continue;
                if (b_mn ? ((bn / 64) % pm != 0) : ((bn / pm) % 8 != 0)) continue;
                if (a_mn && (BM / 64) % pn != 0) continue;
                const int cl = pm * pn;
                const int slots = cl > 1 ? max_clusters(cl, sms) * cl : sms;
                if (slots <= 0) continue;
                const long long tiles = (long long)((num_mb + pm - 1) / pm) * ((num_n + pn - 1) / pn) * cl;
                const int max_s = reduce ? 16 : (num_k >= 128 ? 4 : 1);
                for (int s = 1; s <= max_s; ++s) {
                    if (splits_req > 0 && s != 1) break;
                    int sp = splits_req > 0 ? splits_req : s;
                    if (sp > num_k) sp = num_k;
                    const int kbs = (num_k + sp - 1) / sp;
                    if (splits_req <= 0 && s > 1 && kbs < 8) break;
                    const int s_eff = (num_k + kbs - 1) / kbs;
                    if (splits_req <= 0 && s_eff != s) continue;
                    const long long units = tiles * s_eff;
                    const long long waves = (units + slots - 1) / slots;
                    const double feed = (A_BYTES / (double)pn + bn * BK * 2 / (double)pm) / 64.0;
                    const double mma = 4.0 * bn;
                    const double per_kb = feed > mma ? feed : mma;
                    const double epi = 128.0 * bn * 2.0 / 16.0 + 800.0;
                    const double unit = kbs * per_kb + 600.0 + epi;
                    double cost = waves * unit + 1000.0 * (cl > 1);
                    if (reduce && s_eff > 1) cost += 0.05 * unit * s_eff + (double)M * N * s_eff * 4.0 / 3000.0;
                    if (!reduce && s_eff > 1) cost += 3000.0 + (double)M * N * 2.0 / 2000.0 + (double)M * N * s_eff * 4.0 / 3000.0;
                    if (cost < best) { best = cost; bc = Config{bn, s_eff, pm, pn}; }
                }
            }
        }
    }
    return bc;
}

static int tile_band(int M, int K, int bn_cols, int num_sn) {
    static int l2_cache[64] = {0};
    int dev = 0;
    if (cudaGetDevice(&dev) != cudaSuccess || dev < 0 || dev >= 64) { cudaGetLastError(); return num_sn; }
    if (l2_cache[dev] == 0) {
        int l2 = 0;
        if (cudaDeviceGetAttribute(&l2, cudaDevAttrL2CacheSize, dev) != cudaSuccess || l2 <= 0) { cudaGetLastError(); l2 = -1; }
        l2_cache[dev] = l2;
    }
    const double l2 = (double)l2_cache[dev];
    if (l2 <= 0 || (double)M * K * 2.0 > l2 / 3.0) return num_sn;
    const long long g = (long long)(l2 / 8.0 / ((double)bn_cols * K * 2.0));
    return (int)(g < 1 ? 1 : (g > num_sn ? num_sn : g));
}

struct GatherArgs {
    const void* const* peers;
    int n_peers;
    const int* tile_owner;
    uint32_t* flags;
    uint32_t* epoch;
    uint32_t* done;
};

static int launch(const void* a, long long lda, int a_mn, const void* b, long long ldb, int b_mn, void* d, long long ldd, const void* bias, int M,
                  int N, int K, int accumulate, int bn_req, int splits_req, int pm_req, int pn_req, int msub_req, const GatherArgs* ga, int sms,
                  cudaStream_t st) {
    if (M <= 0 || N <= 0 || K <= 0) return -1;
    if ((lda % 8) || (ldb % 8) || (ldd % 8) || (N % 8)) return -1;
    if (((uintptr_t)a % 16) || ((uintptr_t)b % 16) || ((uintptr_t)d % 16) || (bias && ((uintptr_t)bias % 16))) return -1;
    if (msub_req > 1) return -1;
    int rc = init_once();
    if (rc) return rc;
    const int gather = (ga && ga->n_peers > 0) ? 1 : 0;
    if (gather && (ga->n_peers > MAX_PEERS || a_mn || b_mn || accumulate)) return -1;
    if (bn_req > 0 && bn_req != 64 && bn_req != 128 && bn_req != 256) return -1;
    if ((pm_req > 2) || (pn_req > 2)) return -1;
    Config cfgc{BN_MAX, 1, 1, 1};
    if (!gather) {
        if (g_pm > 0 && pm_req <= 0) pm_req = g_pm;
        if (g_pn > 0 && pn_req <= 0) pn_req = g_pn;
        cfgc = choose_config(M, N, K, a_mn, b_mn, accumulate, sms, bn_req, splits_req, pm_req, pn_req);
    }
    const int bn = cfgc.bn, pm = cfgc.pm, pn = cfgc.pn;
    int splits = cfgc.splits;
    if ((bn_req > 0 && bn != bn_req) || (pm_req > 0 && pm != pm_req) || (pn_req > 0 && pn != pn_req)) return -1;
    if (b_mn ? ((bn / 64) % pm != 0) : ((bn / pm) % 8 != 0)) return -1;
    if (a_mn && (BM / 64) % pn != 0) return -1;
    Params P;
    if (a_mn) rc = make_map(&P.map_a, a, (uint64_t)M, (uint64_t)K, (uint64_t)lda, 64, BK);
    else rc = make_map(&P.map_a, a, (uint64_t)K, (uint64_t)M, (uint64_t)lda, BK, (uint32_t)(BM / pn));
    if (rc) return rc;
    if (b_mn) rc = make_map(&P.map_b, b, (uint64_t)N, (uint64_t)K, (uint64_t)ldb, 64, BK);
    else rc = make_map(&P.map_b, b, (uint64_t)K, (uint64_t)N, (uint64_t)ldb, BK, (uint32_t)(bn / pm));
    if (rc) return rc;
    for (int i = 0; i < MAX_PEERS; ++i) {
        if (gather && i < ga->n_peers) {
            rc = make_map(&P.map_b_peer[i], ga->peers[i], (uint64_t)K, (uint64_t)N, (uint64_t)ldb, BK, (uint32_t)bn);
            if (rc) return rc;
        } else {
            P.map_b_peer[i] = P.map_b;
        }
    }
    rc = make_map(&P.map_d, d, (uint64_t)N, (uint64_t)M, (uint64_t)ldd, 64, 64);
    if (rc) return rc;
    P.bias = (const __nv_bfloat16*)bias;
    P.out = (__nv_bfloat16*)d;
    P.ldd = ldd;
    P.dbg = g_dbg;
    P.tile_owner = gather ? ga->tile_owner : nullptr;
    P.flags = gather ? ga->flags : nullptr;
    P.epoch = gather ? ga->epoch : nullptr;
    P.done_ctas = gather ? ga->done : nullptr;
    P.M = M; P.N = N; P.K = K;
    const int num_k = (K + BK - 1) / BK;
    if (splits < 1) splits = 1;
    if (splits > num_k) splits = num_k;
    P.kb_per_split = (num_k + splits - 1) / splits;
    P.splits = (num_k + P.kb_per_split - 1) / P.kb_per_split;
    P.reduce = accumulate ? 1 : 0;
    bool pdl = g_pdl != 0;
    if (P.splits > 1 && !P.reduce) {
        if (cudaMemset2DAsync(d, (size_t)ldd * 2, 0, (size_t)N * 2, (size_t)M, st) != cudaSuccess) return -6;
        P.reduce = 1;
        pdl = false;
    }
    P.atomic = P.splits > 1 ? 1 : 0;
    P.gather = gather;
    P.pm = pm; P.pn = pn;
    P.stage_bytes = A_BYTES + bn * BK * 2;
    P.stages = RING_BYTES / P.stage_bytes;
    if (P.stages > MAX_STAGES) P.stages = MAX_STAGES;
    const int num_n = (N + bn - 1) / bn;
    const int num_mb = (M + BM - 1) / BM;
    const int cl = pm * pn;
    const int num_sn = (num_n + pn - 1) / pn;
    const long long units = (long long)((num_mb + pm - 1) / pm) * num_sn * P.splits;
    const int slots = cl > 1 ? max_clusters(cl, sms) : sms;
    if (slots <= 0) return -5;
    P.band = gather ? num_sn : tile_band(M, K, bn * pn, num_sn);
    const int grid = (int)(units < (long long)slots ? units : (long long)slots) * cl;
    cudaLaunchConfig_t cfg = {};
    cfg.gridDim = dim3(grid);
    cfg.blockDim = dim3(THREADS);
    cfg.dynamicSmemBytes = SMEM_BYTES;
    cfg.stream = st;
    cudaLaunchAttribute attr[2];
    int na = 0;
    if (cl > 1) {
        attr[na].id = cudaLaunchAttributeClusterDimension;
        attr[na].val.clusterDim.x = cl;
        attr[na].val.clusterDim.y = 1;
        attr[na].val.clusterDim.z = 1;
        ++na;
    }
    if (pdl) {
        attr[na].id = cudaLaunchAttributeProgrammaticStreamSerialization;
        attr[na].val.programmaticStreamSerializationAllowed = 1;
        ++na;
    }
    cfg.attrs = attr;
    cfg.numAttrs = na;
    return (int)cudaLaunchKernelEx(&cfg, kernel_for(bn, a_mn, b_mn), P);
}

}

extern "C" int acco_gemm_run(const void* a, long long lda, int a_mn, const void* b, long long ldb, int b_mn, void* d, long long ldd, const void* bias,
                             int M, int N, int K, int accumulate, int bn_req, int splits_req, int pm_req, int pn_req, int msub_req, int sms,
                             cudaStream_t st) {
    return acco_gemm::launch(a, lda, a_mn, b, ldb, b_mn, d, ldd, bias, M, N, K, accumulate, bn_req, splits_req, pm_req, pn_req, msub_req, nullptr, sms,
                             st);
}

extern "C" int acco_gemm_tn_gather(const void* x, const void* w_local, void* y, int M, int N, int K, const void* const* peers, int n_peers,
                                   const int* tile_owner, uint32_t* flags, uint32_t* epoch, uint32_t* done, int sms, cudaStream_t st) {
    acco_gemm::GatherArgs ga{peers, n_peers, tile_owner, flags, epoch, done};
    return acco_gemm::launch(x, K, 0, w_local, K, 0, y, N, nullptr, M, N, K, 0, 0, 0, 0, 0, 0, n_peers > 0 ? &ga : nullptr, sms, st);
}

extern "C" int acco_gemm_tile_n() { return acco_gemm::BN_MAX; }
extern "C" int acco_gemm_tile_k() { return acco_gemm::BK; }
extern "C" long long acco_gemm_map_encodes() { return acco_gemm::g_map_encodes; }
extern "C" void acco_gemm_set_debug(unsigned long long* buf) { acco_gemm::g_dbg = buf; }
extern "C" int acco_gemm_max_clusters(int cl, int sms) {
    acco_gemm::init_once();
    return acco_gemm::max_clusters(cl, sms);
}
extern "C" void acco_gemm_choose(int M, int N, int K, int a_mn, int b_mn, int accumulate, int sms, int* out5) {
    const acco_gemm::Config c = acco_gemm::choose_config(M, N, K, a_mn, b_mn, accumulate, sms, 0, 0, acco_gemm::g_pm, acco_gemm::g_pn);
    out5[0] = c.bn; out5[1] = c.splits; out5[2] = c.pm; out5[3] = c.pn; out5[4] = 1;
}
```

### acco_b200/models/llama.py

```python
from __future__ import annotations

from collections import OrderedDict
from dataclasses import dataclass, asdict
from typing import Any, Dict, Optional

import torch
import torch.nn as nn

from .. import ops
from .output import CausalLMOutput

__all__ = ["LlamaConfig", "LlamaForCausalLM"]


@dataclass
class LlamaConfig:
    vocab_size: int = 50257
    hidden_size: int = 768
    intermediate_size: int = 2048
    num_hidden_layers: int = 12
    num_attention_heads: int = 12
    num_key_value_heads: Optional[int] = None
    max_position_embeddings: int = 1024
    rms_norm_eps: float = 1e-5
    rope_theta: float = 10000.0
    rope_scaling: Optional[Dict[str, Any]] = None
    tie_word_embeddings: bool = True
    initializer_range: float = 0.02
    pad_vocab_multiple: int = 128
    model_type: str = "llama"

    def __post_init__(self):
        if self.num_key_value_heads is None:
            self.num_key_value_heads = self.num_attention_heads
        assert self.hidden_size % self.num_attention_heads == 0
        assert self.num_attention_heads % self.num_key_value_heads == 0

    @property
    def head_dim(self) -> int:
        return self.hidden_size // self.num_attention_heads

    @property
    def padded_vocab(self) -> int:
        m = max(int(self.pad_vocab_multiple), 1)
        return ((self.vocab_size + m - 1) // m) * m

    def to_dict(self) -> Dict[str, Any]:
        return asdict(self)

    @classmethod
    def from_dict(cls, d: Dict[str, Any]) -> "LlamaConfig":
        keys = cls.__dataclass_fields__.keys()
        return cls(**{k: v for k, v in dict(d).items() if k in keys})

    def num_parameters(self, padded: bool = False) -> int:
        H, I, L = self.hidden_size, self.intermediate_size, self.num_hidden_layers
        D, Hq, Hk = self.head_dim, self.num_attention_heads, self.num_key_value_heads
        V = self.padded_vocab if padded else self.vocab_size
        per_layer = (Hq + 2 * Hk) * D * H + H * Hq * D + 3 * H * I + 2 * H
        n = V * H + L * per_layer + H
        if not self.tie_word_embeddings:
            n += V * H
        return n

    def flops_per_token(self, seq_len: int) -> float:
        H, I, L = self.hidden_size, self.intermediate_size, self.num_hidden_layers
        D, Hq, Hk = self.head_dim, self.num_attention_heads, self.num_key_value_heads
        mm = L * ((Hq + 2 * Hk) * D * H + Hq * D * H + 3 * H * I) + self.vocab_size * H
        attn = L * 2 * Hq * D * seq_len / 2
        return 3.0 * 2.0 * (mm + attn)


class _Norm(nn.Module):
    def __init__(self, dim: int):
        super().__init__()
        self.weight = nn.Parameter(torch.ones(dim))


class _Attn(nn.Module):
    def __init__(self, cfg: LlamaConfig):
        super().__init__()
        D, Hq, Hk, H = cfg.head_dim, cfg.num_attention_heads, cfg.num_key_value_heads, cfg.hidden_size
        self.qkv_proj = nn.Parameter(torch.empty((Hq + 2 * Hk) * D, H))
        self.o_proj = nn.Parameter(torch.empty(H, Hq * D))


class _MLP(nn.Module):
    def __init__(self, cfg: LlamaConfig):
        super().__init__()
        self.gate_up_proj = nn.Parameter(torch.empty(2 * cfg.intermediate_size, cfg.hidden_size))
        self.down_proj = nn.Parameter(torch.empty(cfg.hidden_size, cfg.intermediate_size))


class _Layer(nn.Module):
    def __init__(self, cfg: LlamaConfig):
        super().__init__()
        self.input_layernorm = _Norm(cfg.hidden_size)
        self.self_attn = _Attn(cfg)
        self.post_attention_layernorm = _Norm(cfg.hidden_size)
        self.mlp = _MLP(cfg)


class _Body(nn.Module):
    def __init__(self, cfg: LlamaConfig):
        super().__init__()
        self.embed_tokens = nn.Parameter(torch.empty(cfg.padded_vocab, cfg.hidden_size))
        self.layers = nn.ModuleList([_Layer(cfg) for _ in range(cfg.num_hidden_layers)])
        self.norm = _Norm(cfg.hidden_size)


class LlamaForCausalLM(nn.Module):
    def __init__(self, config: LlamaConfig):
        super().__init__()
        self.config = config
        self.model = _Body(config)
        if config.tie_word_embeddings:
            self.lm_head = None
        else:
            self.lm_head = nn.Parameter(torch.empty(config.padded_vocab, config.hidden_size))
        self._rope_cache: Dict[Any, Any] = {}
        self._ag_table: Dict[int, Any] = {}
        self._ag_idx = 0
        self._ag_pending = False
        self.reset_parameters()

    @torch.no_grad()
    def reset_parameters(self) -> None:
        std = self.config.initializer_range
        V = self.config.vocab_size
        for name, p in self.named_parameters():
            if name.endswith("layernorm.weight") or name.endswith("norm.weight"):
                p.fill_(1.0)
            else:
                p.normal_(0.0, std)
        self.model.embed_tokens[V:].zero_()
        if self.lm_head is not None:
            self.lm_head[V:].zero_()

    @property
    def head_weight(self) -> torch.Tensor:
        return self.model.embed_tokens if self.lm_head is None else self.lm_head

    def num_parameters(self) -> int:
        return sum(p.numel() for p in self.parameters())

    def _rope(self, S: int, device) -> Any:
        key = (S, str(device))
        if key not in self._rope_cache:
            self._rope_cache[key] = ops.rope_tables(S, self.config.head_dim, self.config.rope_theta, device, scaling=self.config.rope_scaling)
        return self._rope_cache[key]

    def fused_ag_candidates(self):
        out = []
        for layer in self.model.layers:
            out += [layer.self_attn.qkv_proj, layer.self_attn.o_proj, layer.mlp.gate_up_proj, layer.mlp.down_proj]
        if self.lm_head is not None:
            out.append(self.lm_head)
        return out

    def _gw(self, p):
        if not self._ag_pending:
            return None
        e = self._ag_table.get(id(p))
        return None if e is None else e[self._ag_idx]

    def forward(self, input_ids: torch.Tensor, attention_mask: Optional[torch.Tensor] = None,
                labels: Optional[torch.Tensor] = None, position_ids: Optional[torch.Tensor] = None, **unused) -> CausalLMOutput:
        cfg = self.config
        B, S = input_ids.shape
        T = B * S
        D, Hq, Hk = cfg.head_dim, cfg.num_attention_heads, cfg.num_key_value_heads
        cos, sin = self._rope(S, input_ids.device)
        seg = None
        if position_ids is not None:
            pos = position_ids.reshape(T)
            cos, sin = cos[pos], sin[pos]
            seg = ops.segment_starts(position_ids)
        eps = cfg.rms_norm_eps

        h = ops.embedding(input_ids.reshape(T), self.model.embed_tokens)
        branch = None
        for layer in self.model.layers:
            if branch is None:
                n = ops.rmsnorm(h, layer.input_layernorm.weight, eps)
            else:
                n, h = ops.add_rmsnorm(branch, h, layer.input_layernorm.weight, eps)
            qkv = ops.linear(n, layer.self_attn.qkv_proj, gathered=self._gw(layer.self_attn.qkv_proj))
            att = ops.rope_causal_attention(qkv, cos, sin, B, S, Hq, Hk, D, seg=seg)
            o = ops.linear(att, layer.self_attn.o_proj, gathered=self._gw(layer.self_attn.o_proj))
            n, h = ops.add_rmsnorm(o, h, layer.post_attention_layernorm.weight, eps)
            gu = ops.linear(n, layer.mlp.gate_up_proj, gathered=self._gw(layer.mlp.gate_up_proj))
            branch = ops.linear(ops.swiglu(gu), layer.mlp.down_proj, gathered=self._gw(layer.mlp.down_proj))
        if branch is None:
            n = ops.rmsnorm(h, self.model.norm.weight, eps)
        else:
            n, h = ops.add_rmsnorm(branch, h, self.model.norm.weight, eps)
        logits = ops.linear(n, self.head_weight, gathered=self._gw(self.head_weight) if self.lm_head is not None else None)
        if labels is None:
            return CausalLMOutput(loss=None, logits=logits.view(B, S, -1)[..., : cfg.vocab_size])
        shifted = torch.full_like(labels, -100)
        shifted[:, :-1] = labels[:, 1:]
        loss = ops.softmax_cross_entropy(logits, shifted.reshape(T), cfg.vocab_size, -100)
        return CausalLMOutput(loss=loss, logits=None)

    def state_dict(self, *args, destination=None, prefix: str = "", keep_vars: bool = False, **kw):
        cfg = self.config
        D, Hq, Hk, V, I = cfg.head_dim, cfg.num_attention_heads, cfg.num_key_value_heads, cfg.vocab_size, cfg.intermediate_size
        get = (lambda p: p) if keep_vars else (lambda p: p.detach())
        sd = destination if destination is not None else OrderedDict()
        sd[prefix + "model.embed_tokens.weight"] = get(self.model.embed_tokens)[:V]
        for i, layer in enumerate(self.model.layers):
            base = f"{prefix}model.layers.{i}."
            qkv = get(layer.self_attn.qkv_proj)
            sd[base + "self_attn.q_proj.weight"] = qkv[: Hq * D]
            sd[base + "self_attn.k_proj.weight"] = qkv[Hq * D: (Hq + Hk) * D]
            sd[base + "self_attn.v_proj.weight"] = qkv[(Hq + Hk) * D:]
            sd[base + "self_attn.o_proj.weight"] = get(layer.self_attn.o_proj)
            gu = get(layer.mlp.gate_up_proj)
            sd[base + "mlp.gate_proj.weight"] = gu[:I]
            sd[base + "mlp.up_proj.weight"] = gu[I:]
            sd[base + "mlp.down_proj.weight"] = get(layer.mlp.down_proj)
            sd[base + "input_layernorm.weight"] = get(layer.input_layernorm.weight)
            sd[base + "post_attention_layernorm.weight"] = get(layer.post_attention_layernorm.weight)
        sd[prefix + "model.norm.weight"] = get(self.model.norm.weight)
        sd[prefix + "lm_head.weight"] = get(self.head_weight)[:V]
        return sd

    @torch.no_grad()
    def load_state_dict(self, state_dict, strict: bool = True, assign: bool = False):
        cfg = self.config
        D, Hq, Hk, V, I = cfg.head_dim, cfg.num_attention_heads, cfg.num_key_value_heads, cfg.vocab_size, cfg.intermediate_size
        sd = dict(state_dict)
        used = set()

        def take(name):
            used.add(name)
            return sd[name]

        missing = []

        def put(dst: torch.Tensor, name: str):
            if name in sd:
                dst.copy_(take(name).to(dst.dtype))
            else:
                missing.append(name)

        put(self.model.embed_tokens[:V], "model.embed_tokens.weight")
        for i, layer in enumerate(self.model.layers):
            b = f"model.layers.{i}."
            qkv, gu = layer.self_attn.qkv_proj, layer.mlp.gate_up_proj
            put(qkv[: Hq * D], b + "self_attn.q_proj.weight")
            put(qkv[Hq * D: (Hq + Hk) * D], b + "self_attn.k_proj.weight")
            put(qkv[(Hq + Hk) * D:], b + "self_attn.v_proj.weight")
            put(layer.self_attn.o_proj, b + "self_attn.o_proj.weight")
            put(gu[:I], b + "mlp.gate_proj.weight")
            put(gu[I:], b + "mlp.up_proj.weight")
            put(layer.mlp.down_proj, b + "mlp.down_proj.weight")
            put(layer.input_layernorm.weight, b + "input_layernorm.weight")
            put(layer.post_attention_layernorm.weight, b + "post_attention_layernorm.weight")
        put(self.model.norm.weight, "model.norm.weight")
        if self.lm_head is not None:
            put(self.lm_head[:V], "lm_head.weight")
        elif "lm_head.weight" in sd:
            used.add("lm_head.weight")
        unexpected = [k for k in sd if k not in used and not k.endswith("rotary_emb.inv_freq")]
        if strict and (missing or unexpected):
            raise RuntimeError(f"load_state_dict: missing={missing[:5]} unexpected={unexpected[:5]}")
        return torch.nn.modules.module._IncompatibleKeys(missing, unexpected)
```

### acco_b200/ops/__init__.py

```python
from __future__ import annotations

import glob
import importlib.util
import os
import threading
from typing import Dict, Optional

import torch

_EXT = None
_EXT_ERR: Optional[BaseException] = None
_LOCK = threading.Lock()
_PKG_DIR = os.path.dirname(os.path.dirname(os.path.abspath(__file__)))

_launch_counts: Dict[str, int] = {}
_counting = True


def count_launch(name: str, n: int = 1) -> None:
    if _counting:
        _launch_counts[name] = _launch_counts.get(name, 0) + n


def launch_counts() -> Dict[str, int]:
    return dict(_launch_counts)


def reset_launch_counts() -> None:
    _launch_counts.clear()


def total_launches() -> int:
    return sum(_launch_counts.values())


def ext_path() -> Optional[str]:
    cands = sorted(glob.glob(os.path.join(_PKG_DIR, "_C*.so")))
    return cands[-1] if cands else None


def load_ext(required: bool = False):
    global _EXT, _EXT_ERR
    if _EXT is not None:
        return _EXT
    with _LOCK:
        if _EXT is not None:
            return _EXT
        path = ext_path()
        if path is None:
            _EXT_ERR = FileNotFoundError(
                f"acco_b200/_C*.so not found under {_PKG_DIR}; run `python -c 'import __graft_entry__ as g; g.build()'`")
        else:
            try:
                spec = importlib.util.spec_from_file_location("acco_b200._C", path)
                mod = importlib.util.module_from_spec(spec)
                spec.loader.exec_module(mod)
                _EXT = mod
                _EXT_ERR = None
            except BaseException as e:
                _EXT_ERR = e
        if _EXT is None and required:
            raise RuntimeError(f"acco_b200 CUDA extension unavailable: {_EXT_ERR}")
        return _EXT


def have_ext() -> bool:
    return load_ext() is not None


def use_kernels(*tensors: torch.Tensor, bf16_only: bool = True) -> bool:
    if not tensors or not all(t.is_cuda for t in tensors if t is not None):
        return False
    if bf16_only and any(t.is_floating_point() and t.dtype != torch.bfloat16 for t in tensors if t is not None):
        return False
    if os.environ.get("ACCO_FORCE_EAGER") == "1":
        return False
    if load_ext() is not None:
        return True
    if os.environ.get("ACCO_ALLOW_FALLBACK") == "1":
        return False
    raise RuntimeError(
        "acco_b200: CUDA tensors given but the sm_90a extension is not built/loaded "
        f"({_EXT_ERR}). Build it with __graft_entry__.build() or set ACCO_ALLOW_FALLBACK=1.")


from .norm import rmsnorm, add_rmsnorm, rmsnorm_ref, add_rmsnorm_ref
from .layernorm import layernorm, add_layernorm, gelu_new, layernorm_ref, add_layernorm_ref, gelu_new_ref
from .rope import rope_qkv, rope_qkv_ref, apply_rope_ref, rope_tables
from .embedding import embedding
from .swiglu import swiglu, swiglu_ref
from .cross_entropy import softmax_cross_entropy, softmax_cross_entropy_ref
from .linear import linear, LinearFn
from .attention import causal_attention, causal_attention_ref, rope_causal_attention, packed_causal_attention, segment_starts
from .adam import fused_adamw_shard, grad_sumsq

__all__ = [
    "load_ext", "have_ext", "use_kernels", "ext_path",
    "count_launch", "launch_counts", "reset_launch_counts", "total_launches",
    "rmsnorm", "add_rmsnorm", "rmsnorm_ref", "add_rmsnorm_ref",
    "layernorm", "add_layernorm", "gelu_new", "layernorm_ref", "add_layernorm_ref", "gelu_new_ref",
    "rope_qkv", "rope_qkv_ref", "apply_rope_ref", "rope_tables", "embedding",
    "swiglu", "swiglu_ref",
    "softmax_cross_entropy", "softmax_cross_entropy_ref",
    "linear", "LinearFn",
    "causal_attention", "causal_attention_ref", "rope_causal_attention", "packed_causal_attention", "segment_starts",
    "fused_adamw_shard", "grad_sumsq",
]
```

### acco_b200/ops/gemm.py

```python
from __future__ import annotations

from typing import List

import torch

from . import count_launch, load_ext, use_kernels

TILE_N, TILE_K = 256, 64


def gemm_tn_ref(x: torch.Tensor, w: torch.Tensor) -> torch.Tensor:
    return (x.float() @ w.float().t()).to(x.dtype)


def _rowmajor(t: torch.Tensor) -> torch.Tensor:
    if t.dim() == 2 and t.stride(1) == 1 and t.stride(0) % 8 == 0 and t.stride(0) >= t.shape[1] and t.data_ptr() % 16 == 0:
        return t
    return t.contiguous()


def gemm_supported(*mats: torch.Tensor) -> bool:
    return all(m.is_cuda and m.dtype == torch.bfloat16 and m.dim() == 2 and m.shape[1] % 8 == 0 and m.shape[0] > 0 for m in mats)


def gemm_ref(a, b, out=None, bias=None, a_mn=False, b_mn=False, accumulate=False):
    af = (a.t() if a_mn else a).float()
    bf = (b.t() if b_mn else b).float()
    y = af @ bf.t()
    if bias is not None:
        y = y + bias.float()
    if accumulate:
        y = y + out.float()
    y = y.to(a.dtype)
    if out is not None:
        out.copy_(y)
        return out
    return y


def gemm(a: torch.Tensor, b: torch.Tensor, out: torch.Tensor = None, bias: torch.Tensor = None, a_mn: bool = False, b_mn: bool = False,
         accumulate: bool = False, bn: int = 0, splits: int = 0, pm: int = 0, pn: int = 0, msub: int = 0, max_ctas: int = 0) -> torch.Tensor:
    if not use_kernels(a, b):
        return gemm_ref(a, b, out, bias, a_mn, b_mn, accumulate)
    y = load_ext(required=True).gemm(_rowmajor(a), _rowmajor(b), out, bias, bool(a_mn), bool(b_mn), bool(accumulate), int(bn), int(splits),
                                     int(pm), int(pn), int(msub), int(max_ctas))
    count_launch("gemm")
    return y


def gemm_tn(x: torch.Tensor, w: torch.Tensor, max_ctas: int = 0, bias: torch.Tensor = None) -> torch.Tensor:
    return gemm(x, w, bias=bias, max_ctas=max_ctas)


def gemm_nn(dy: torch.Tensor, w: torch.Tensor) -> torch.Tensor:
    return gemm(dy, w, b_mn=True)


def gemm_tt_acc(dy: torch.Tensor, x: torch.Tensor, grad: torch.Tensor) -> torch.Tensor:
    return gemm(dy, x, out=grad, a_mn=True, b_mn=True, accumulate=True)


class GatheredWeight:

    def __init__(self, n: int, k: int, offset: int, peer_bases: List[int], size_slice: int, rank: int, device):
        self.n, self.k, self.offset, self.rank = int(n), int(k), int(offset), int(rank)
        self.peer_ptrs = [int(b) + 2 * self.offset for b in peer_bases]
        num_n = (self.n + TILE_N - 1) // TILE_N
        num_k = (self.k + TILE_K - 1) // TILE_K
        owners = []
        for t in range(num_n):
            lo = self.offset + t * TILE_N * self.k
            hi = self.offset + min((t + 1) * TILE_N, self.n) * self.k - 1
            o_lo, o_hi = lo // size_slice, hi // size_slice
            owners.append(o_lo if (o_lo == o_hi and o_lo != rank) else -1)
        self.owners = owners
        self.tile_owner = torch.tensor(owners, dtype=torch.int32, device=device)
        self.flags = torch.zeros(num_n * num_k * 2, dtype=torch.int32, device=device)
        self.state = torch.zeros(2, dtype=torch.int32, device=device)

    def pulled_ranges(self, for_rank: int, size_slice: int):
        out = []
        for t in range((self.n + TILE_N - 1) // TILE_N):
            lo = self.offset + t * TILE_N * self.k
            hi = self.offset + min((t + 1) * TILE_N, self.n) * self.k
            if lo // size_slice == (hi - 1) // size_slice == for_rank:
                out.append((lo, hi))
        return out


def gemm_tn_gather(x: torch.Tensor, w_local: torch.Tensor, gw: GatheredWeight, max_ctas: int = 0) -> torch.Tensor:
    out = load_ext(required=True).gemm_tn(x.contiguous(), w_local, gw.peer_ptrs, gw.tile_owner, gw.flags, gw.state, int(max_ctas))
    count_launch("gemm_gather")
    return out
```

### acco_b200/ops/linear.py

```python
from __future__ import annotations

from typing import Optional

import os

import torch
import torch.nn.functional as F


def _tc(*mats) -> bool:
    from . import use_kernels
    from .gemm import gemm_supported
    if os.environ.get("ACCO_GEMM", "") == "cublas":
        return False
    return use_kernels(*mats) and gemm_supported(*mats)


class LinearFn(torch.autograd.Function):
    @staticmethod
    @torch.amp.custom_fwd(device_type="cuda")
    def forward(ctx, x, weight, bias, accumulate_into_grad):
        ctx.save_for_backward(x, weight)
        ctx.has_bias = bias is not None
        ctx.accumulate = bool(accumulate_into_grad)
        ctx.weight_ref = weight
        ctx.bias_ref = bias
        x2 = x.reshape(-1, x.shape[-1])
        if _tc(x2, weight) and (bias is None or (bias.dtype == torch.bfloat16 and bias.data_ptr() % 16 == 0)):
            from .gemm import gemm_tn
            return gemm_tn(x2, weight.detach(), bias=None if bias is None else bias.detach()).view(*x.shape[:-1], weight.shape[0])
        return F.linear(x, weight, bias)

    @staticmethod
    @torch.amp.custom_bwd(device_type="cuda")
    def backward(ctx, dy):
        return _linear_backward(ctx, dy)


_SIDE_STREAMS = {}


def _wgrad_stream(device):
    if os.environ.get("ACCO_WGRAD_STREAM", "0") != "1" or device.type != "cuda":
        return None
    key = (device.index, torch.cuda.current_stream(device).cuda_stream)
    st = _SIDE_STREAMS.get(key)
    if st is None:
        st = _SIDE_STREAMS[key] = torch.cuda.Stream(device=device)
    return st


def _linear_backward(ctx, dy):
    x, weight = ctx.saved_tensors
    dy2 = dy.reshape(-1, dy.shape[-1])
    x2 = x.reshape(-1, x.shape[-1])
    if dy2.dtype != weight.dtype or x2.dtype != dy2.dtype:
        weight_c, x2 = weight.to(dy2.dtype), x2.to(dy2.dtype)
    else:
        weight_c = weight
    tc = _tc(dy2, weight_c, x2)
    w = ctx.weight_ref
    acc_tc = (ctx.needs_input_grad[1] and ctx.accumulate and w.grad is not None and tc and w.grad.dtype == torch.bfloat16
              and w.grad.dim() == 2 and w.grad.stride(1) == 1 and w.grad.data_ptr() % 16 == 0)
    dx = dw = db = None
    side = _wgrad_stream(dy2.device) if (acc_tc and ctx.needs_input_grad[0]) else None
    if side is not None:
        from .gemm import gemm_tt_acc
        cur = torch.cuda.current_stream(dy2.device)
        side.wait_stream(cur)
        with torch.cuda.stream(side):
            gemm_tt_acc(dy2, x2, w.grad)
        dy2.record_stream(side)
        x2.record_stream(side)
    if ctx.needs_input_grad[0]:
        if tc:
            from .gemm import gemm_nn
            dx = gemm_nn(dy2, weight_c.detach()).view(x.shape)
        else:
            dx = dy2.matmul(weight_c).view(x.shape).to(x.dtype)
    if side is not None:
        torch.cuda.current_stream(dy2.device).wait_stream(side)
    elif ctx.needs_input_grad[1]:
        if ctx.accumulate and w.grad is not None:
            if acc_tc:
                from .gemm import gemm_tt_acc
                gemm_tt_acc(dy2, x2, w.grad)
            elif w.grad.dtype == dy2.dtype:
                w.grad.addmm_(dy2.t(), x2)
            else:
                w.grad.add_(dy2.t().matmul(x2))
        elif tc:
            from .gemm import gemm
            dw = gemm(dy2, x2, a_mn=True, b_mn=True)
        else:
            dw = dy2.t().matmul(x2).to(weight.dtype)
    if ctx.has_bias and ctx.needs_input_grad[2]:
        b = ctx.bias_ref
        if ctx.accumulate and b.grad is not None:
            b.grad.add_(dy2.sum(0))
        else:
            db = dy2.sum(0).to(b.dtype)
    return dx, dw, db, None


class GatherLinearFn(torch.autograd.Function):

    @staticmethod
    def forward(ctx, x, weight, gathered, accumulate_into_grad):
        from .gemm import gemm_tn_gather
        ctx.save_for_backward(x, weight)
        ctx.has_bias = False
        ctx.accumulate = bool(accumulate_into_grad)
        ctx.weight_ref = weight
        ctx.bias_ref = None
        x2 = x.reshape(-1, x.shape[-1])
        return gemm_tn_gather(x2, weight.detach(), gathered).view(*x.shape[:-1], weight.shape[0])

    @staticmethod
    def backward(ctx, dy):
        dx, dw, _db, _ = _linear_backward(ctx, dy)
        return dx, dw, None, None


def linear(x: torch.Tensor, weight: torch.Tensor, bias: Optional[torch.Tensor] = None, accumulate_into_grad: bool = True,
           gathered=None) -> torch.Tensor:
    if gathered is not None and bias is None and x.is_cuda:
        if torch.is_grad_enabled() and (weight.requires_grad or x.requires_grad):
            return GatherLinearFn.apply(x, weight, gathered, accumulate_into_grad)
        from .gemm import gemm_tn_gather
        x2 = x.reshape(-1, x.shape[-1])
        return gemm_tn_gather(x2, weight.detach(), gathered).view(*x.shape[:-1], weight.shape[0])
    if torch.is_grad_enabled() and (weight.requires_grad or x.requires_grad):
        return LinearFn.apply(x, weight, bias, accumulate_into_grad)
    return F.linear(x, weight, bias)
```

### acco_b200/ops/swiglu.py

```python
from __future__ import annotations

import torch
import torch.nn.functional as F

from . import count_launch, load_ext, use_kernels


def swiglu_ref(gate_up: torch.Tensor) -> torch.Tensor:
    g, u = gate_up.float().chunk(2, dim=-1)
    return (F.silu(g) * u).to(gate_up.dtype)


class _SwiGLUFn(torch.autograd.Function):
    @staticmethod
    def forward(ctx, gate_up):
        C = load_ext(required=True)
        gu = gate_up.reshape(-1, gate_up.shape[-1]).contiguous()
        out = C.swiglu_fwd(gu)
        count_launch("swiglu_fwd")
        ctx.save_for_backward(gu)
        ctx.shape = gate_up.shape
        return out.view(*gate_up.shape[:-1], gate_up.shape[-1] // 2)

    @staticmethod
    def backward(ctx, dout):
        C = load_ext(required=True)
        (gu,) = ctx.saved_tensors
        d = dout.reshape(-1, dout.shape[-1]).contiguous()
        dgu = C.swiglu_bwd(d, gu)
        count_launch("swiglu_bwd")
        return dgu.view(ctx.shape)


def swiglu(gate_up: torch.Tensor) -> torch.Tensor:
    if use_kernels(gate_up):
        return _SwiGLUFn.apply(gate_up)
    return swiglu_ref(gate_up)
```

Measured before the change: 312,800.

## Fuse SwiGLU activation into gate-up GEMM epilogue and its gradient into down-proj dgrad

Adds two WGMMA kernel variants. One computes the gate_up projection and applies SwiGLU in the epilogue, writing both gu and the activation. The other computes the down-projection input gradient and applies the SwiGLU backward in the epilogue, reading gu via TMA. A new autograd function routes the Llama MLP through these kernels, which removes the standalone elementwise swiglu launches and their extra HBM round-trips. The cost is a smaller smem ring for the dswiglu variant, fixed tile shapes, and falling back to the unfused path when weights are gathered.

```diff
diff --git a/acco_b200/csrc/bindings.cpp b/acco_b200/csrc/bindings.cpp
--- a/acco_b200/csrc/bindings.cpp
+++ b/acco_b200/csrc/bindings.cpp
@@ -36,6 +36,8 @@
                   int M, int N, int K, int accumulate, int bn_req, int splits_req, int pm_req, int pn_req, int msub_req, int sms, cudaStream_t st);
 int acco_gemm_tn_gather(const void* x, const void* w_local, void* y, int M, int N, int K, const void* const* peers, int n_peers,
                         const int* tile_owner, uint32_t* flags, uint32_t* epoch, uint32_t* done, int sms, cudaStream_t st);
+int acco_gemm_swiglu(const void* x, const void* w, void* gu, void* act, int M, int I, int K, int sms, cudaStream_t st);
+int acco_gemm_dswiglu(const void* dy, const void* w, const void* gu, void* dgu, int M, int I, int K, int sms, cudaStream_t st);
 long long acco_gemm_map_encodes();
 int acco_gemm_max_clusters(int cl, int sms);
 void acco_gemm_set_debug(unsigned long long* buf);
@@ -462,6 +464,30 @@
     return y;
 }
 
+std::vector<torch::Tensor> gemm_swiglu(torch::Tensor x, torch::Tensor w) {
+    check_bf16(x, "x"); check_bf16(w, "w_gate_up");
+    TORCH_CHECK(x.dim() == 2 && w.dim() == 2 && x.size(1) == w.size(1) && w.size(0) % 256 == 0, "gemm_swiglu: x [T,H], w [2I,H], I % 128 == 0");
+    const c10::cuda::CUDAGuard guard(x.device());
+    const int64_t T = x.size(0), H = x.size(1), I = w.size(0) / 2;
+    auto gu = torch::empty({T, 2 * I}, x.options());
+    auto act = torch::empty({T, I}, x.options());
+    const int rc = acco_gemm_swiglu(x.data_ptr(), w.data_ptr(), gu.data_ptr(), act.data_ptr(), (int)T, (int)I, (int)H, sm_count(), stream());
+    TORCH_CHECK(rc == 0, "gemm_swiglu launch failed, code ", rc, " (T=", T, " I=", I, " H=", H, ")");
+    return {gu, act};
+}
+
+torch::Tensor gemm_dswiglu(torch::Tensor dy, torch::Tensor w, torch::Tensor gu) {
+    check_bf16(dy, "dy"); check_bf16(w, "w_down"); check_bf16(gu, "gate_up");
+    TORCH_CHECK(dy.dim() == 2 && w.dim() == 2 && gu.dim() == 2 && dy.size(1) == w.size(0) && w.size(1) % 128 == 0 && gu.size(0) == dy.size(0) &&
+                gu.size(1) == 2 * w.size(1), "gemm_dswiglu: dy [T,H], w [H,I], gu [T,2I], I % 128 == 0");
+    const c10::cuda::CUDAGuard guard(dy.device());
+    const int64_t T = dy.size(0), H = dy.size(1), I = w.size(1);
+    auto dgu = torch::empty_like(gu);
+    const int rc = acco_gemm_dswiglu(dy.data_ptr(), w.data_ptr(), gu.data_ptr(), dgu.data_ptr(), (int)T, (int)I, (int)H, sm_count(), stream());
+    TORCH_CHECK(rc == 0, "gemm_dswiglu launch failed, code ", rc, " (T=", T, " I=", I, " H=", H, ")");
+    return dgu;
+}
+
 std::vector<int64_t> gemm_choose(int64_t M, int64_t N, int64_t K, bool a_mn, bool b_mn, bool accumulate) {
     int o[5] = {0, 0, 0, 0, 0};
     acco_gemm_choose((int)M, (int)N, (int)K, a_mn ? 1 : 0, b_mn ? 1 : 0, accumulate ? 1 : 0, sm_count(), o);
@@ -565,6 +591,8 @@
           py::arg("mode"), py::arg("grid"), py::arg("max_norm"));
     m.def("gemm_tn", &gemm_tn);
     m.def("gemm", &gemm);
+    m.def("gemm_swiglu", &gemm_swiglu);
+    m.def("gemm_dswiglu", &gemm_dswiglu);
     m.def("gemm_choose", &gemm_choose);
     m.def("gemm_map_encodes", &gemm_map_encodes);
     m.def("gemm_max_clusters", &gemm_max_clusters);
diff --git a/acco_b200/csrc/elementwise.cu b/acco_b200/csrc/elementwise.cu
--- a/acco_b200/csrc/elementwise.cu
+++ b/acco_b200/csrc/elementwise.cu
@@ -1,6 +1,7 @@
 #include <stdlib.h>
 
 #include "common.cuh"
+#include "swiglu.cuh"
 
 namespace acco {
 
@@ -101,10 +102,7 @@
         unpack8(ld_stream(g), fg);
         unpack8(ld_stream(g + I), fu);
 #pragma unroll
-        for (int j = 0; j < 8; ++j) {
-            const float sg = 1.f / (1.f + __expf(-fg[j]));
-            o[j] = fg[j] * sg * fu[j];
-        }
+        for (int j = 0; j < 8; ++j) o[j] = swiglu_act(fg[j], fu[j]);
         st_stream(out + t * I + 8 * v, pack8(o));
     }
 }
@@ -124,12 +122,7 @@
         unpack8(ld_stream(g + I), fu);
         unpack8(ld_stream(dout + t * I + 8 * v), fd);
 #pragma unroll
-        for (int j = 0; j < 8; ++j) {
-            const float sg = 1.f / (1.f + __expf(-fg[j]));
-            const float silu = fg[j] * sg;
-            dg[j] = fd[j] * fu[j] * sg * (1.f + fg[j] * (1.f - sg));
-            du[j] = fd[j] * silu;
-        }
+        for (int j = 0; j < 8; ++j) swiglu_grad(fg[j], fu[j], fd[j], dg[j], du[j]);
         __nv_bfloat16* o = dgu + t * 2 * I + 8 * v;
         st_stream(o, pack8(dg));
         st_stream(o + I, pack8(du));
diff --git a/acco_b200/csrc/gemm_wgmma.cu b/acco_b200/csrc/gemm_wgmma.cu
--- a/acco_b200/csrc/gemm_wgmma.cu
+++ b/acco_b200/csrc/gemm_wgmma.cu
@@ -7,6 +7,7 @@
 #include <mutex>
 #include <unordered_map>
 
+#include "swiglu.cuh"
 #include "wgmma.cuh"
 
 namespace acco_gemm {
@@ -23,6 +24,7 @@
 constexpr int THREADS = 384;
 constexpr int MAX_PEERS = 8;
 constexpr int MN_CHUNK_BYTES = 64 * BK * 2;
+constexpr int EPI_PLAIN = 0, EPI_SWIGLU = 1, EPI_DSWIGLU = 2;
 
 struct Params {
     CUtensorMap map_a;
@@ -45,6 +47,7 @@
     int pm, pn;
     int band;
     unsigned long long* dbg;
+    CUtensorMap map_e;
 };
 
 __device__ __forceinline__ void wait_flag_gpu(const uint32_t* f, uint32_t epoch) {
@@ -95,13 +98,16 @@
     else wgmma_m64n64k16<TA, TB>(acc, da, db, scale_d);
 }
 
-template <int BN, int A_MN, int B_MN>
-__global__ void __launch_bounds__(THREADS, 1) gemm_kernel(const __grid_constant__ Params P) {
+template <int BN, int A_MN, int B_MN, int EPI>
+__device__ __forceinline__ void gemm_body(const Params& P) {
     extern __shared__ uint8_t smem_raw[];
     if (threadIdx.x == 0) stamp(P, 0);
+    constexpr int TN = EPI == EPI_SWIGLU ? BN / 2 : BN;
+    constexpr int RING = EPI == EPI_DSWIGLU ? RING_BYTES - EPI_BYTES : RING_BYTES;
+    constexpr int EPI_SZ = EPI == EPI_DSWIGLU ? 2 * EPI_BYTES : EPI_BYTES;
     uint8_t* smem = (uint8_t*)(((uintptr_t)smem_raw + 1023) & ~(uintptr_t)1023);
-    uint8_t* epi_smem = smem + RING_BYTES;
-    uint64_t* full_bar = (uint64_t*)(epi_smem + EPI_BYTES);
+    uint8_t* epi_smem = smem + RING;
+    uint64_t* full_bar = (uint64_t*)(epi_smem + EPI_SZ);
     uint64_t* empty_bar = full_bar + MAX_STAGES;
     uint64_t* c_bar = empty_bar + MAX_STAGES;
 
@@ -112,7 +118,7 @@
     const uint32_t cl_rank = cl_size > 1 ? cluster_ctarank() : 0u;
     const int pi = (int)cl_rank / pn, pj = (int)cl_rank - pi * pn;
     const int unit0 = blockIdx.x / cl_size, unit_stride = gridDim.x / cl_size;
-    const int num_n = (P.N + BN - 1) / BN, num_k = (P.K + BK - 1) / BK, num_mb = (P.M + BM - 1) / BM;
+    const int num_n = (P.N + TN - 1) / TN, num_k = (P.K + BK - 1) / BK, num_mb = (P.M + BM - 1) / BM;
     const int num_sn = (num_n + pn - 1) / pn, num_smb = (num_mb + pm - 1) / pm;
     const int band = P.band;
     const int tiles = num_smb * num_sn;
@@ -127,6 +133,7 @@
         asm volatile("prefetch.tensormap [%0];" ::"l"(&P.map_a) : "memory");
         asm volatile("prefetch.tensormap [%0];" ::"l"(&P.map_b) : "memory");
         asm volatile("prefetch.tensormap [%0];" ::"l"(&P.map_d) : "memory");
+        if (EPI != EPI_PLAIN) asm volatile("prefetch.tensormap [%0];" ::"l"(&P.map_e) : "memory");
         for (int s = 0; s < n_stages; ++s) {
             mbar_init(&full_bar[s], 1);
             mbar_init(&empty_bar[s], 2u * (uint32_t)(pm + pn - 1));
@@ -188,7 +195,10 @@
                         if (mc_a) tma_load_2d_mc(&P.map_a, &full_bar[stage], sa + a_off * 128, kb * BK, m0 + a_off, mask_a);
                         else tma_load_2d(&P.map_a, &full_bar[stage], sa, kb * BK, m0);
                     }
-                    if (B_MN) {
+                    if (EPI == EPI_SWIGLU) {
+                        tma_load_2d(bmap, &full_bar[stage], sb, kb * BK, n_blk * TN);
+                        tma_load_2d(bmap, &full_bar[stage], sb + TN * 128, kb * BK, P.N + n_blk * TN);
+                    } else if (B_MN) {
                         for (int c = b_ch0; c < b_ch0 + nbch; ++c) {
                             if (mc_b) tma_load_2d_mc(bmap, &full_bar[stage], sb + c * MN_CHUNK_BYTES, n0 + c * 64, kb * BK, mask_b);
                             else tma_load_2d(bmap, &full_bar[stage], sb + c * MN_CHUNK_BYTES, n0 + c * 64, kb * BK);
@@ -227,7 +237,7 @@
         };
         constexpr int NSUB = BN / 64;
         constexpr int NPRE = NSUB < 2 ? NSUB : 2;
-        uint8_t* epi = epi_smem + cw * 2 * EPI_BUF_BYTES;
+        uint8_t* epi = epi_smem + cw * (EPI_SZ / EPI_BYTES) * 2 * EPI_BUF_BYTES;
         uint64_t* cbar = c_bar + cw * 2;
         const bool load_c = P.reduce && !P.atomic;
         const int bar_id = 1 + cw;
@@ -240,6 +250,12 @@
             mbar_expect_tx(&cbar[s & 1], (uint32_t)EPI_BUF_BYTES);
             tma_load_2d(&P.map_d, &cbar[s & 1], epi + (s & 1) * EPI_BUF_BYTES, u.n_blk * BN + s * 64, u.mb * BM + cw * 64);
         };
+        auto load_gu_sub = [&](const Unit& u, int s) {
+            const int c = u.n_blk * BN + s * 64, r = u.mb * BM + cw * 64;
+            mbar_expect_tx(&cbar[s], (uint32_t)(2 * EPI_BUF_BYTES));
+            tma_load_2d(&P.map_e, &cbar[s], epi + 2 * s * EPI_BUF_BYTES, c, r);
+            tma_load_2d(&P.map_e, &cbar[s], epi + (2 * s + 1) * EPI_BUF_BYTES, P.N + c, r);
+        };
         float acc[BN / 2];
 #pragma unroll
         for (int i = 0; i < BN / 2; ++i) acc[i] = 0.f;
@@ -261,6 +277,10 @@
                     mma_k16<BN, A_MN, B_MN>(acc, da, db, (uint32_t)((kb > u.kb0) | (k != 0)));
                 }
                 wgmma_commit();
+                if (EPI == EPI_DSWIGLU && kb == u.kb0 && tid == 0) {
+                    bulk_wait_read<0>();
+                    for (int s = 0; s < NSUB; ++s) load_gu_sub(u, s);
+                }
                 if (load_c && kb == u.kb0 && tid == 0) {
                     bulk_wait_read<0>();
                     for (int s = 0; s < NPRE; ++s) load_c_sub(u, s);
@@ -277,6 +297,80 @@
             release(prev);
             const int m0 = u.mb * BM + cw * 64;
             const uint32_t row_addr = smem_u32(epi) + (uint32_t)((warp * 16 + (lane >> 2)) * 128 + 4 * (lane & 3));
+            if constexpr (EPI == EPI_SWIGLU) {
+#pragma unroll
+                for (int s = 0; s < 6; ++s) {
+                    const int q = s / 3, kind = s % 3;
+                    uint8_t* buf = epi + (s & 1) * EPI_BUF_BYTES;
+                    const uint32_t buf_addr = row_addr + (uint32_t)((s & 1) * EPI_BUF_BYTES);
+                    const uint32_t up_addr = row_addr + (uint32_t)(((s + 1) & 1) * EPI_BUF_BYTES);
+                    if (tid == 0) bulk_wait_read<1>();
+                    named_barrier(bar_id, 128);
+#pragma unroll
+                    for (int jj = 0; jj < 8; ++jj) {
+                        const uint32_t off = (uint32_t)((jj ^ (lane >> 2)) << 4);
+#pragma unroll
+                        for (int h = 0; h < 2; ++h) {
+                            const uint32_t o = off + h * 8 * 128;
+                            if (kind < 2) {
+                                const int j = kind * 16 + q * 8 + jj;
+                                st_shared_u32(buf_addr + o, pack_bf16x2(acc[4 * j + 2 * h], acc[4 * j + 2 * h + 1]));
+                            } else {
+                                const uint32_t gv = ld_shared_u32(buf_addr + o), uv = ld_shared_u32(up_addr + o);
+                                const float2 g = __bfloat1622float2(*reinterpret_cast<const __nv_bfloat162*>(&gv));
+                                const float2 up = __bfloat1622float2(*reinterpret_cast<const __nv_bfloat162*>(&uv));
+                                st_shared_u32(buf_addr + o, pack_bf16x2(acco::swiglu_act(g.x, up.x), acco::swiglu_act(g.y, up.y)));
+                            }
+                        }
+                    }
+                    fence_async_smem();
+                    named_barrier(bar_id, 128);
+                    if (tid == 0) {
+                        const int c = u.n_blk * TN + q * 64;
+                        if (kind == 0) tma_store_2d(&P.map_d, buf, c, m0);
+                        else if (kind == 1) tma_store_2d(&P.map_d, buf, P.N + c, m0);
+                        else tma_store_2d(&P.map_e, buf, c, m0);
+                        bulk_commit();
+                    }
+                }
+                continue;
+            }
+            if constexpr (EPI == EPI_DSWIGLU) {
+#pragma unroll
+                for (int s = 0; s < NSUB; ++s) {
+                    mbar_wait(&cbar[s], c_phase);
+                    const uint32_t g_addr = row_addr + (uint32_t)(2 * s * EPI_BUF_BYTES), u_addr = g_addr + EPI_BUF_BYTES;
+#pragma unroll
+                    for (int jj = 0; jj < 8; ++jj) {
+                        const uint32_t off = (uint32_t)((jj ^ (lane >> 2)) << 4);
+#pragma unroll
+                        for (int h = 0; h < 2; ++h) {
+                            const int j = s * 8 + jj;
+                            const uint32_t o = off + h * 8 * 128;
+                            const uint32_t gv = ld_shared_u32(g_addr + o), uv = ld_shared_u32(u_addr + o);
+                            const uint32_t dv = pack_bf16x2(acc[4 * j + 2 * h], acc[4 * j + 2 * h + 1]);
+                            const float2 g = __bfloat1622float2(*reinterpret_cast<const __nv_bfloat162*>(&gv));
+                            const float2 up = __bfloat1622float2(*reinterpret_cast<const __nv_bfloat162*>(&uv));
+                            const float2 d = __bfloat1622float2(*reinterpret_cast<const __nv_bfloat162*>(&dv));
+                            float dg0, du0, dg1, du1;
+                            acco::swiglu_grad(g.x, up.x, d.x, dg0, du0);
+                            acco::swiglu_grad(g.y, up.y, d.y, dg1, du1);
+                            st_shared_u32(g_addr + o, pack_bf16x2(dg0, dg1));
+                            st_shared_u32(u_addr + o, pack_bf16x2(du0, du1));
+                        }
+                    }
+                    fence_async_smem();
+                    named_barrier(bar_id, 128);
+                    if (tid == 0) {
+                        const int c = u.n_blk * BN + s * 64;
+                        tma_store_2d(&P.map_d, epi + 2 * s * EPI_BUF_BYTES, c, m0);
+                        tma_store_2d(&P.map_d, epi + (2 * s + 1) * EPI_BUF_BYTES, P.N + c, m0);
+                        bulk_commit();
+                    }
+                }
+                c_phase ^= 1u;
+                continue;
+            }
             const int colb = u.n_blk * BN + 2 * (lane & 3);
             const bool bias_on = P.bias != nullptr && u.kb0 == 0;
 #pragma unroll
@@ -342,6 +436,13 @@
         }
     }
 }
+
+template <int BN, int A_MN, int B_MN>
+__global__ void __launch_bounds__(THREADS, 1) gemm_kernel(const __grid_constant__ Params P) {
+    gemm_body<BN, A_MN, B_MN, EPI_PLAIN>(P);
+}
+__global__ void __launch_bounds__(THREADS, 1) gemm_swiglu_kernel(const __grid_constant__ Params P) { gemm_body<256, 0, 0, EPI_SWIGLU>(P); }
+__global__ void __launch_bounds__(THREADS, 1) gemm_dswiglu_kernel(const __grid_constant__ Params P) { gemm_body<128, 0, 1, EPI_DSWIGLU>(P); }
 
 typedef CUresult (*EncodeFn)(CUtensorMap*, CUtensorMapDataType, cuuint32_t, void*, const cuuint64_t*, const cuuint64_t*, const cuuint32_t*,
                              const cuuint32_t*, CUtensorMapInterleave, CUtensorMapSwizzle, CUtensorMapL2promotion, CUtensorMapFloatOOBfill);
@@ -450,6 +551,8 @@
             for (int a = 0; a < 2; ++a)
                 for (int b = 0; b < 2; ++b)
                     if (cudaFuncSetAttribute(kernel_for(bn, a, b), cudaFuncAttributeMaxDynamicSharedMemorySize, SMEM_BYTES) != cudaSuccess) rc = -4;
+        for (KernelFn f : {gemm_swiglu_kernel, gemm_dswiglu_kernel})
+            if (cudaFuncSetAttribute(f, cudaFuncAttributeMaxDynamicSharedMemorySize, SMEM_BYTES) != cudaSuccess) rc = -4;
         const char* e;
         if ((e = getenv("ACCO_GEMM_CLUSTER")) && e[0] && e[1] == ',') { g_pm = e[0] - '0'; g_pn = e[2] - '0'; }
         if ((e = getenv("ACCO_GEMM_PDL")) && e[0] == '0') g_pdl = 0;
@@ -560,6 +663,8 @@
     uint32_t* done;
 };
 
+static int launch_kernel(KernelFn fn, const Params& P, int grid, int cl, bool pdl, cudaStream_t st);
+
 static int launch(const void* a, long long lda, int a_mn, const void* b, long long ldb, int b_mn, void* d, long long ldd, const void* bias, int M,
                   int N, int K, int accumulate, int bn_req, int splits_req, int pm_req, int pn_req, int msub_req, const GatherArgs* ga, int sms,
                   cudaStream_t st) {
@@ -637,6 +742,51 @@
     if (slots <= 0) return -5;
     P.band = gather ? num_sn : tile_band(M, K, bn * pn, num_sn);
     const int grid = (int)(units < (long long)slots ? units : (long long)slots) * cl;
+    return launch_kernel(kernel_for(bn, a_mn, b_mn), P, grid, cl, pdl, st);
+}
+
+static int launch_swiglu(int epi, const void* a, const void* b, void* d, void* e, int M, int I, int K, int sms, cudaStream_t st) {
+    if (M <= 0 || I <= 0 || K <= 0 || (I % 128) || (K % 8)) return -1;
+    if (((uintptr_t)a % 16) || ((uintptr_t)b % 16) || ((uintptr_t)d % 16) || ((uintptr_t)e % 16)) return -1;
+    int rc = init_once();
+    if (rc) return rc;
+    const bool fwd = epi == EPI_SWIGLU;
+    const int bn = fwd ? 256 : 128;
+    Params P;
+    rc = make_map(&P.map_a, a, (uint64_t)K, (uint64_t)M, (uint64_t)K, BK, BM);
+    if (!rc) rc = fwd ? make_map(&P.map_b, b, (uint64_t)K, 2ull * I, (uint64_t)K, BK, 128)
+                      : make_map(&P.map_b, b, (uint64_t)I, (uint64_t)K, (uint64_t)I, 64, BK);
+    if (!rc) rc = make_map(&P.map_d, d, 2ull * I, (uint64_t)M, 2ull * I, 64, 64);
+    if (!rc) rc = fwd ? make_map(&P.map_e, e, (uint64_t)I, (uint64_t)M, (uint64_t)I, 64, 64) : make_map(&P.map_e, e, 2ull * I, (uint64_t)M, 2ull * I, 64, 64);
+    if (rc) return rc;
+    for (int i = 0; i < MAX_PEERS; ++i) P.map_b_peer[i] = P.map_b;
+    P.bias = nullptr;
+    P.tile_owner = nullptr;
+    P.flags = nullptr;
+    P.epoch = nullptr;
+    P.done_ctas = nullptr;
+    P.out = (__nv_bfloat16*)d;
+    P.ldd = 2ll * I;
+    P.M = M; P.N = I; P.K = K;
+    const int num_k = (K + BK - 1) / BK;
+    P.splits = 1;
+    P.kb_per_split = num_k;
+    P.reduce = 0;
+    P.atomic = 0;
+    P.gather = 0;
+    P.pm = 1; P.pn = 1;
+    P.stage_bytes = A_BYTES + bn * BK * 2;
+    P.stages = (fwd ? RING_BYTES : RING_BYTES - EPI_BYTES) / P.stage_bytes;
+    if (P.stages > MAX_STAGES) P.stages = MAX_STAGES;
+    P.dbg = g_dbg;
+    const int num_n = I / 128, num_mb = (M + BM - 1) / BM;
+    const long long units = (long long)num_mb * num_n;
+    P.band = tile_band(M, K, bn, num_n);
+    const int grid = (int)(units < (long long)sms ? units : (long long)sms);
+    return launch_kernel(fwd ? gemm_swiglu_kernel : gemm_dswiglu_kernel, P, grid, 1, g_pdl != 0, st);
+}
+
+static int launch_kernel(KernelFn fn, const Params& P, int grid, int cl, bool pdl, cudaStream_t st) {
     cudaLaunchConfig_t cfg = {};
     cfg.gridDim = dim3(grid);
     cfg.blockDim = dim3(THREADS);
@@ -658,7 +808,7 @@
     }
     cfg.attrs = attr;
     cfg.numAttrs = na;
-    return (int)cudaLaunchKernelEx(&cfg, kernel_for(bn, a_mn, b_mn), P);
+    return (int)cudaLaunchKernelEx(&cfg, fn, P);
 }
 
 }
@@ -674,6 +824,14 @@
                                    const int* tile_owner, uint32_t* flags, uint32_t* epoch, uint32_t* done, int sms, cudaStream_t st) {
     acco_gemm::GatherArgs ga{peers, n_peers, tile_owner, flags, epoch, done};
     return acco_gemm::launch(x, K, 0, w_local, K, 0, y, N, nullptr, M, N, K, 0, 0, 0, 0, 0, 0, n_peers > 0 ? &ga : nullptr, sms, st);
+}
+
+extern "C" int acco_gemm_swiglu(const void* x, const void* w, void* gu, void* act, int M, int I, int K, int sms, cudaStream_t st) {
+    return acco_gemm::launch_swiglu(acco_gemm::EPI_SWIGLU, x, w, gu, act, M, I, K, sms, st);
+}
+
+extern "C" int acco_gemm_dswiglu(const void* dy, const void* w, const void* gu, void* dgu, int M, int I, int K, int sms, cudaStream_t st) {
+    return acco_gemm::launch_swiglu(acco_gemm::EPI_DSWIGLU, dy, w, dgu, const_cast<void*>(gu), M, I, K, sms, st);
 }
 
 extern "C" int acco_gemm_tile_n() { return acco_gemm::BN_MAX; }
diff --git a/acco_b200/csrc/swiglu.cuh b/acco_b200/csrc/swiglu.cuh
--- /dev/null
+++ b/acco_b200/csrc/swiglu.cuh
@@ -0,0 +1,16 @@
+#pragma once
+#include <cuda_runtime.h>
+
+namespace acco {
+
+__device__ __forceinline__ float swiglu_sigmoid(float g) { return 1.f / (1.f + __expf(-g)); }
+
+__device__ __forceinline__ float swiglu_act(float g, float u) { return __fmul_rn(__fmul_rn(g, swiglu_sigmoid(g)), u); }
+
+__device__ __forceinline__ void swiglu_grad(float g, float u, float d, float& dg, float& du) {
+    const float sg = swiglu_sigmoid(g);
+    dg = __fmul_rn(__fmul_rn(__fmul_rn(d, u), sg), __fmaf_rn(g, 1.f - sg, 1.f));
+    du = __fmul_rn(d, __fmul_rn(g, sg));
+}
+
+}
diff --git a/acco_b200/models/llama.py b/acco_b200/models/llama.py
--- a/acco_b200/models/llama.py
+++ b/acco_b200/models/llama.py
@@ -189,8 +189,8 @@
             att = ops.rope_causal_attention(qkv, cos, sin, B, S, Hq, Hk, D, seg=seg)
             o = ops.linear(att, layer.self_attn.o_proj, gathered=self._gw(layer.self_attn.o_proj))
             n, h = ops.add_rmsnorm(o, h, layer.post_attention_layernorm.weight, eps)
-            gu = ops.linear(n, layer.mlp.gate_up_proj, gathered=self._gw(layer.mlp.gate_up_proj))
-            branch = ops.linear(ops.swiglu(gu), layer.mlp.down_proj, gathered=self._gw(layer.mlp.down_proj))
+            branch = ops.swiglu_mlp(n, layer.mlp.gate_up_proj, layer.mlp.down_proj, gathered_gate_up=self._gw(layer.mlp.gate_up_proj),
+                                    gathered_down=self._gw(layer.mlp.down_proj))
         if branch is None:
             n = ops.rmsnorm(h, self.model.norm.weight, eps)
         else:
diff --git a/acco_b200/ops/__init__.py b/acco_b200/ops/__init__.py
--- a/acco_b200/ops/__init__.py
+++ b/acco_b200/ops/__init__.py
@@ -88,7 +88,7 @@
 from .layernorm import layernorm, add_layernorm, gelu_new, layernorm_ref, add_layernorm_ref, gelu_new_ref
 from .rope import rope_qkv, rope_qkv_ref, apply_rope_ref, rope_tables
 from .embedding import embedding
-from .swiglu import swiglu, swiglu_ref
+from .swiglu import swiglu, swiglu_ref, swiglu_mlp
 from .cross_entropy import softmax_cross_entropy, softmax_cross_entropy_ref
 from .linear import linear, LinearFn
 from .attention import causal_attention, causal_attention_ref, rope_causal_attention, packed_causal_attention, segment_starts
@@ -100,7 +100,7 @@
     "rmsnorm", "add_rmsnorm", "rmsnorm_ref", "add_rmsnorm_ref",
     "layernorm", "add_layernorm", "gelu_new", "layernorm_ref", "add_layernorm_ref", "gelu_new_ref",
     "rope_qkv", "rope_qkv_ref", "apply_rope_ref", "rope_tables", "embedding",
-    "swiglu", "swiglu_ref",
+    "swiglu", "swiglu_ref", "swiglu_mlp",
     "softmax_cross_entropy", "softmax_cross_entropy_ref",
     "linear", "LinearFn",
     "causal_attention", "causal_attention_ref", "rope_causal_attention", "packed_causal_attention", "segment_starts",
diff --git a/acco_b200/ops/gemm.py b/acco_b200/ops/gemm.py
--- a/acco_b200/ops/gemm.py
+++ b/acco_b200/ops/gemm.py
@@ -60,6 +60,18 @@
     return gemm(dy, x, out=grad, a_mn=True, b_mn=True, accumulate=True)
 
 
+def gemm_swiglu(x: torch.Tensor, w_gate_up: torch.Tensor):
+    gu, act = load_ext(required=True).gemm_swiglu(x, w_gate_up)
+    count_launch("gemm_swiglu")
+    return gu, act
+
+
+def gemm_dswiglu(dy: torch.Tensor, w_down: torch.Tensor, gu: torch.Tensor) -> torch.Tensor:
+    dgu = load_ext(required=True).gemm_dswiglu(dy, w_down, gu)
+    count_launch("gemm_dswiglu")
+    return dgu
+
+
 class GatheredWeight:
 
     def __init__(self, n: int, k: int, offset: int, peer_bases: List[int], size_slice: int, rank: int, device):
diff --git a/acco_b200/ops/linear.py b/acco_b200/ops/linear.py
--- a/acco_b200/ops/linear.py
+++ b/acco_b200/ops/linear.py
@@ -52,6 +52,12 @@
 
 def _linear_backward(ctx, dy):
     x, weight = ctx.saved_tensors
+    dx, dw, db = _linear_grads(dy, x, weight, ctx.weight_ref, ctx.accumulate, ctx.needs_input_grad[0], ctx.needs_input_grad[1],
+                               ctx.bias_ref if ctx.has_bias and ctx.needs_input_grad[2] else None)
+    return dx, dw, db, None
+
+
+def _linear_grads(dy, x, weight, w, accumulate, need_dx, need_dw, bias=None, dgrad=None):
     dy2 = dy.reshape(-1, dy.shape[-1])
     x2 = x.reshape(-1, x.shape[-1])
     if dy2.dtype != weight.dtype or x2.dtype != dy2.dtype:
@@ -59,11 +65,10 @@
     else:
         weight_c = weight
     tc = _tc(dy2, weight_c, x2)
-    w = ctx.weight_ref
-    acc_tc = (ctx.needs_input_grad[1] and ctx.accumulate and w.grad is not None and tc and w.grad.dtype == torch.bfloat16
+    acc_tc = (need_dw and accumulate and w.grad is not None and tc and w.grad.dtype == torch.bfloat16
               and w.grad.dim() == 2 and w.grad.stride(1) == 1 and w.grad.data_ptr() % 16 == 0)
     dx = dw = db = None
-    side = _wgrad_stream(dy2.device) if (acc_tc and ctx.needs_input_grad[0]) else None
+    side = _wgrad_stream(dy2.device) if (acc_tc and need_dx) else None
     if side is not None:
         from .gemm import gemm_tt_acc
         cur = torch.cuda.current_stream(dy2.device)
@@ -72,16 +77,18 @@
             gemm_tt_acc(dy2, x2, w.grad)
         dy2.record_stream(side)
         x2.record_stream(side)
-    if ctx.needs_input_grad[0]:
-        if tc:
+    if need_dx:
+        if dgrad is not None:
+            dx = dgrad(dy2, weight_c.detach())
+        elif tc:
             from .gemm import gemm_nn
             dx = gemm_nn(dy2, weight_c.detach()).view(x.shape)
         else:
             dx = dy2.matmul(weight_c).view(x.shape).to(x.dtype)
     if side is not None:
         torch.cuda.current_stream(dy2.device).wait_stream(side)
-    elif ctx.needs_input_grad[1]:
-        if ctx.accumulate and w.grad is not None:
+    elif need_dw:
+        if accumulate and w.grad is not None:
             if acc_tc:
                 from .gemm import gemm_tt_acc
                 gemm_tt_acc(dy2, x2, w.grad)
@@ -94,13 +101,12 @@
             dw = gemm(dy2, x2, a_mn=True, b_mn=True)
         else:
             dw = dy2.t().matmul(x2).to(weight.dtype)
-    if ctx.has_bias and ctx.needs_input_grad[2]:
-        b = ctx.bias_ref
-        if ctx.accumulate and b.grad is not None:
-            b.grad.add_(dy2.sum(0))
+    if bias is not None:
+        if accumulate and bias.grad is not None:
+            bias.grad.add_(dy2.sum(0))
         else:
-            db = dy2.sum(0).to(b.dtype)
-    return dx, dw, db, None
+            db = dy2.sum(0).to(bias.dtype)
+    return dx, dw, db
 
 
 class GatherLinearFn(torch.autograd.Function):
diff --git a/acco_b200/ops/swiglu.py b/acco_b200/ops/swiglu.py
--- a/acco_b200/ops/swiglu.py
+++ b/acco_b200/ops/swiglu.py
@@ -36,3 +36,62 @@
     if use_kernels(gate_up):
         return _SwiGLUFn.apply(gate_up)
     return swiglu_ref(gate_up)
+
+
+class _SwiGLUMLPFn(torch.autograd.Function):
+
+    @staticmethod
+    @torch.amp.custom_fwd(device_type="cuda")
+    def forward(ctx, n, w_gate_up, w_down, gathered_gate_up, gathered_down, accumulate_into_grad):
+        from .gemm import gemm_swiglu, gemm_tn, gemm_tn_gather
+        n2 = n.reshape(-1, n.shape[-1])
+        if gathered_gate_up is None:
+            gu, act = gemm_swiglu(n2, w_gate_up.detach())
+        else:
+            gu = gemm_tn_gather(n2, w_gate_up.detach(), gathered_gate_up)
+            act = load_ext(required=True).swiglu_fwd(gu)
+            count_launch("swiglu_fwd")
+        if gathered_down is None:
+            y = gemm_tn(act, w_down.detach())
+        else:
+            y = gemm_tn_gather(act, w_down.detach(), gathered_down)
+        ctx.save_for_backward(n2, gu, act, w_gate_up, w_down)
+        ctx.weight_refs = (w_gate_up, w_down)
+        ctx.accumulate = bool(accumulate_into_grad)
+        ctx.shape = n.shape
+        return y.view(*n.shape[:-1], w_down.shape[0])
+
+    @staticmethod
+    @torch.amp.custom_bwd(device_type="cuda")
+    def backward(ctx, dy):
+        from .gemm import gemm_dswiglu
+        from .linear import _linear_grads
+        n2, gu, act, w_gate_up, w_down = ctx.saved_tensors
+        w_gate_up_ref, w_down_ref = ctx.weight_refs
+        need_n, need_wgu, need_wd = ctx.needs_input_grad[:3]
+        dgu, dwd, _ = _linear_grads(dy, act, w_down, w_down_ref, ctx.accumulate, need_n or need_wgu, need_wd,
+                                    dgrad=lambda dy2, w: gemm_dswiglu(dy2.contiguous(), w, gu))
+        dn = dwgu = None
+        if dgu is not None:
+            dn, dwgu, _ = _linear_grads(dgu, n2, w_gate_up, w_gate_up_ref, ctx.accumulate, need_n, need_wgu)
+        return None if dn is None else dn.view(ctx.shape), dwgu, dwd, None, None, None
+
+
+def _fusable(n: torch.Tensor, w_gate_up: torch.Tensor, w_down: torch.Tensor) -> bool:
+    from .linear import _tc
+    if not (torch.is_grad_enabled() and (n.requires_grad or w_gate_up.requires_grad or w_down.requires_grad)):
+        return False
+    if not (n.is_cuda and w_gate_up.dim() == 2 and w_down.dim() == 2):
+        return False
+    i = w_down.shape[1]
+    return (_tc(n.reshape(-1, n.shape[-1]), w_gate_up, w_down) and i % 128 == 0 and w_gate_up.shape == (2 * i, n.shape[-1])
+            and all(t.is_contiguous() and t.data_ptr() % 16 == 0 for t in (n, w_gate_up, w_down)))
+
+
+def swiglu_mlp(n: torch.Tensor, w_gate_up: torch.Tensor, w_down: torch.Tensor, gathered_gate_up=None, gathered_down=None,
+               accumulate_into_grad: bool = True) -> torch.Tensor:
+    if _fusable(n, w_gate_up, w_down):
+        return _SwiGLUMLPFn.apply(n, w_gate_up, w_down, gathered_gate_up, gathered_down, accumulate_into_grad)
+    from .linear import linear
+    gu = linear(n, w_gate_up, accumulate_into_grad=accumulate_into_grad, gathered=gathered_gate_up)
+    return linear(swiglu(gu), w_down, accumulate_into_grad=accumulate_into_grad, gathered=gathered_down)
```

Measured after the change: 317,900 (median of 6 runs). 1.02x the previous value.
